# Amanda-Zheng/MR-GNAS

Measured on AMD Instinct MI355X. Metric: million edges/sec per supernet fwd+bwd step (FB15k-237, dim=200), higher is better.
Workload: dtype f32

## Files before the change

mr-gnas_amd/csrc/gemm_dispatch.hpp:

```cpp
#pragma once
#include "gemm_x3.hpp"
#include "gemm_x3s.hpp"
#include "gemm_x3s8.hpp"
#include "gemm_x3q.hpp"

namespace mrg {

inline int gemm_mode() { return gemm_switches().mode; }

constexpr int X3Q_MIN_K = 224;
inline bool x3q_shape(int epi, int N, int K) {
  const int q = gemm_switches().q;
  return gemm_mode() == 0 && q != 0 && epi != EPI_SEGMAX && epi != EPI_SEGSUM && N > 128 && N <= X3Q_NT * 16 && K > (q == 2 ? 48 : X3Q_MIN_K);
}

constexpr int X3N_NT = 2;
inline bool x3n_shape(int epi, int64_t rows, int N, int K) {
  return gemm_mode() == 0 && rows > 0 && rows <= gemm_switches().small_rows && gemm_pick_nt(N) > X3N_NT && N <= 224 && !x3q_shape(epi, N, K);
}

inline size_t bsplit_bytes_any(int N, int K) {
  const size_t a = x3_bsplit_bytes(N, K, gemm_pick_nt(N));
  const size_t q = (N > 128 && N <= X3Q_NT * 16) ? x3q_bsplit_bytes(K) : 0;
  const size_t n = (gemm_pick_nt(N) > X3N_NT && N <= 224) ? x3_bsplit_bytes(N, K, X3N_NT) : 0;
  const size_t m = a > q ? a : q;
  return m > n ? m : n;
}

inline void launch_bsplit_any(int epi, int64_t rows, const float* B, int64_t sn, int64_t sk, int N, int K, void* Bp, hipStream_t st) {
  if (x3q_shape(epi, N, K)) {
    const float* Bs[1] = {B};
    void* outs[1] = {Bp};
    launch_bsplitq3(Bs, sn, sk, N, K, outs, 1, st);
  } else {
    launch_bsplit(B, sn, sk, N, K, x3n_shape(epi, rows, N, K) ? X3N_NT : gemm_pick_nt(N), Bp, st);
  }
}
inline void launch_bsplit3_any(int epi, int64_t rows, const float* const* B, int64_t sn, int64_t sk, int N, int K, void* const* out, hipStream_t st,
                               const float* const* B2 = nullptr, int ksplit = 0) {
  if (x3q_shape(epi, N, K)) launch_bsplitq3(B, sn, sk, N, K, out, 3, st, B2, ksplit);
  else launch_bsplit3(B, sn, sk, N, K, x3n_shape(epi, rows, N, K) ? X3N_NT : gemm_pick_nt(N), out, st, B2, ksplit);
}

template <int EPI>
inline int launch_rowgemm_x3_mode(GemmArgs a, const void* Bp, hipStream_t st) {
  if (x3q_shape(EPI, a.N, a.K1 + a.K2)) {
    if (!x3q_eligible(a)) return MRG_E_SHAPE;
    return launch_rowgemm_x3q<EPI>(a, Bp, st);
  }
  if (x3n_shape(EPI, a.rows, a.N, a.K1 + a.K2)) {
    if (!x3_eligible(a)) return MRG_E_SHAPE;
    return launch_rowgemm_x3<EPI>(a, Bp, st, X3N_NT);
  }
  if (gemm_mode() != 2 && x3s_eligible(a)) {
    if constexpr (EPI != EPI_GATE) {
      if (x3s8_eligible<EPI>(a)) return launch_rowgemm_x3s8<EPI>(a, Bp, st);
    }
    return launch_rowgemm_x3s<EPI>(a, Bp, st);
  }
  return launch_rowgemm_x3<EPI>(a, Bp, st);
}

inline size_t gemm_workspace_bytes(int K, int N) {
  const size_t split = bsplit_bytes_any(N, K);
  const size_t transp = (size_t)K * N * sizeof(float);
  return split > transp ? split : transp;
}

template <int EPI>
inline int launch_gemm(GemmArgs a, int64_t b_sn, int64_t b_sk, void* ws, hipStream_t st) {
  if (a.rows <= 0) return MRG_OK;
  if (!a.A2 || a.K2 == 0) { a.A2 = a.A1; a.K2 = 0; }
  const int K = a.K1 + a.K2;
  if (ws && gemm_mode() != 1 && x3_eligible(a)) {
    launch_bsplit_any(EPI, a.rows, a.B, b_sn, b_sk, a.N, K, ws, st);
    return launch_rowgemm_x3_mode<EPI>(a, ws, st);
  }
  if (b_sk != 1) {
    if (!ws) return MRG_E_WORKSPACE;
    launch_transpose(a.B, (float*)ws, (int)(K), a.N, (int)b_sk, st);
    a.B = (const float*)ws;
    a.ldb = K;
  } else {
    a.ldb = (int)b_sn;
  }
  return launch_rowgemm<EPI>(a, st);
}

}
```

mr-gnas_amd/csrc/gemm_x3q.hpp:

```cpp
#pragma once
#include "gemm_x3.hpp"

namespace mrg {

constexpr int X3Q_CHUNK = X3Q_HT * 3 * 1024;
constexpr int X3Q_ROWS = 64;

inline size_t x3q_bsplit_bytes(int K) { return (size_t)x3q_slabs(K) * 2 * X3Q_CHUNK; }

template <int EPI>
__device__ __forceinline__ void gemm_epilogue_q(const GemmArgs& a, f32x4v (&acc)[X3Q_NT], int64_t rowbase, int li, int lh, bool full) {
  if (rowbase >= a.rows) return;
  const int last = (int)((a.rows - 1 - rowbase) < 15 ? (a.rows - 1 - rowbase) : 15);
  const int colw = li < a.N ? li : a.N - 1;
  float* crow[8];
  const float* srow[8];
  float* xrow[8];
  float cs[8];
  bool rok[8];
  const bool cstore = EPI != EPI_GATE || a.C != nullptr;
#pragma unroll
  for (int i = 0; i < 8; ++i) {
    const int row = i + 8 * lh;
    const int rc = row < last ? row : last;
    rok[i] = row <= last;
    crow[i] = a.C + (rowbase + rc) * a.ldc + colw;
    if (EPI == EPI_GATE) srow[i] = a.S + (rowbase + rc) * a.ld_s + colw;
    if (EPI == EPI_ACCUM) srow[i] = a.Cin + (rowbase + rc) * a.ld_cin + colw;
    if (EPI == EPI_GATE) xrow[i] = a.aux ? a.aux + (rowbase + rc) * a.N + colw : nullptr;
    cs[i] = 1.0f;
    if (EPI == EPI_GATE || EPI == EPI_SCALE) cs[i] = a.scale * (a.rowscale ? a.rowscale[rowbase + rc] : 1.0f);
  }
  const int lc = li & 15;
#pragma unroll
  for (int j = 0; j < X3Q_HT; ++j) {
    const int ca = (2 * j) * 16 + lc, cb = (2 * j + 1) * 16 + lc;
    const float bva = a.bias ? a.bias[ca < a.N ? ca : a.N - 1] : 0.f;
    const float bvb = a.bias ? a.bias[cb < a.N ? cb : a.N - 1] : 0.f;
    float acc8[8];
#pragma unroll
    for (int r = 0; r < 4; ++r) {
      float xa = acc[2 * j][r] + bva, xb = acc[2 * j + 1][r] + bvb;
      asm volatile("s_nop 1\n\tv_permlane16_swap_b32 %0, %1" : "+v"(xa), "+v"(xb));
      acc8[r] = xa;
      acc8[4 + r] = xb;
    }
    const int col = j * 32 + li;
    const bool cok = col < a.N;
    const int off = cok ? j * 32 : 0;
    float in[8], v[8], g[8];
#pragma unroll
    for (int i = 0; i < 8; ++i) in[i] = 0.f;
    if ((EPI == EPI_GATE && cstore) || EPI == EPI_ACCUM) {
#pragma unroll
      for (int i = 0; i < 8; ++i) in[i] = srow[i][off];
    }
#pragma unroll
    for (int i = 0; i < 8; ++i) {
      const float x = acc8[i];
      if (EPI == EPI_BIAS_ACT) {
        v[i] = (a.act == MRG_ACT_RELU) ? (x > 0.f ? x : 0.f) : (a.act == MRG_ACT_SIGMOID ? sigmoidf_fast(x) : x);
      } else if (EPI == EPI_GATE) {
        g[i] = sigmoidf_fast(x);
        v[i] = g[i] * in[i] * cs[i];
      } else if (EPI == EPI_SCALE) {
        v[i] = x * cs[i];
      } else {
        v[i] = x + in[i];
      }
    }
    if (full) {
      if (cok) {
        if (cstore) {
#pragma unroll
          for (int i = 0; i < 8; ++i) crow[i][j * 32] = v[i];
        }
        if (EPI == EPI_GATE && a.aux) {
#pragma unroll
          for (int i = 0; i < 8; ++i) xrow[i][j * 32] = g[i];
        }
      }
    } else {
#pragma unroll
      for (int i = 0; i < 8; ++i) {
        if (cok && rok[i]) {
          if (cstore) crow[i][j * 32] = v[i];
          if (EPI == EPI_GATE && a.aux) xrow[i][j * 32] = g[i];
        }
      }
    }
  }
}

constexpr int X3Q_WPS = 3;

template <int EPI, bool DUAL>
__global__ __launch_bounds__(256, X3Q_WPS) void rowgemm_x3q_k(GemmArgs a, const char* __restrict__ Bp) {
  constexpr int NCH = X3Q_HT * 3;
  constexpr int NBW = (NCH + 3) / 4;
  extern __shared__ __align__(16) char smem_q[];
  const int tid = threadIdx.x, wave = __builtin_amdgcn_readfirstlane(tid >> 6), lane = tid & 63;
  const int lr = lane & 15, lg = lane >> 4;
  MRG_GROUP_SELECT(X3Q_ROWS)
  const int64_t roww = row0 + wave * 16;
  const int K = a.K1 + a.K2;
  const int nslab = (K + 31) >> 5;

  f32x4v acc[X3Q_NT];
#pragma unroll
  for (int n = 0; n < X3Q_NT; ++n)
#pragma unroll
    for (int r = 0; r < 4; ++r) acc[n][r] = 0.f;

  const float* ar1; const float* ar2;
  x3_a_row(a, roww + lr, ar1, ar2);
  v4f xr[2][2];
  auto load_a = [&](int slab, v4f (&x)[2]) { x3_load_a<32, DUAL>(x, slab, nslab, lg, ar1, ar2, a.K1, a.K2, K); };
  auto fetch_b = [&](int c) { x3_fetch_b<NCH>(Bq + (int64_t)c * X3Q_CHUNK, smem_q + (c & 1) * X3Q_CHUNK, wave, lane); };
  const unsigned lds0 = (unsigned)(size_t)(lds_ptr_t)smem_q + (unsigned)lane * 16u;
  u32x4 bq[2][3];
  auto read_b = [&](int t, int buf, u32x4 (&q)[3]) { x3_read_b(lds0 + (unsigned)(buf * X3Q_CHUNK + t * 3072), q); };
  u32x4 ch, cm, cl, nh, nm, nl;
  load_a(0, xr[0]);
  fetch_b(0);
  fetch_b(1);
  load_a(1, xr[1]);
  asm volatile("s_waitcnt vmcnt(%0)" ::"n"(NBW + 2) : "memory");
  __builtin_amdgcn_sched_barrier(0);
#pragma unroll
  for (int q = 0; q < 4; ++q) split_pair_of(xr[0], q, ch, cm, cl);
  __builtin_amdgcn_s_barrier();

  auto half_slab = [&](auto half_c, auto split_c, const v4f (&xn)[2]) {
    constexpr int HF = decltype(half_c)::value;
    constexpr bool SPLIT = decltype(split_c)::value;
    read_b(0, HF, bq[0]);
#pragma unroll
    for (int t = 0; t < X3Q_HT; ++t) {
      if (t + 1 < X3Q_HT) {
        read_b(t + 1, HF, bq[(t + 1) & 1]);
        asm volatile("s_waitcnt lgkmcnt(3)" ::: "memory");
      } else {
        asm volatile("s_waitcnt lgkmcnt(0)" ::: "memory");
      }
      __builtin_amdgcn_sched_barrier(0);
      if (SPLIT && t < 4) split_pair_of(xn, t, nh, nm, nl);
      const bf16x8 Ah = __builtin_bit_cast(bf16x8, ch), Am = __builtin_bit_cast(bf16x8, cm), Al = __builtin_bit_cast(bf16x8, cl);
      const bf16x8 Bh = __builtin_bit_cast(bf16x8, bq[t & 1][0]), Bm = __builtin_bit_cast(bf16x8, bq[t & 1][1]), Bl = __builtin_bit_cast(bf16x8, bq[t & 1][2]);
      x3_chain(acc[HF * X3Q_HT + t], Ah, Am, Al, Bh, Bm, Bl);
      if (SPLIT) {
#pragma unroll
        for (int i = 0; i < 6; ++i) {
          __builtin_amdgcn_sched_group_barrier(0x008, 1, 0);
          __builtin_amdgcn_sched_group_barrier(0x002, 2, 0);
        }
      }
      __builtin_amdgcn_sched_barrier(0);
    }
  };

  auto slab = [&](auto r_c, int s) {
    constexpr int R = decltype(r_c)::value;
    const bool has_next = s + 1 < nslab;
    if (s > 0) fetch_b(2 * s + 1);
    half_slab(std::integral_constant<int, 0>{}, std::false_type{}, xr[0]);
    asm volatile("s_waitcnt vmcnt(0)" ::: "memory");
    __builtin_amdgcn_s_barrier();
    if (has_next) fetch_b(2 * s + 2);
    load_a(s + 2, xr[R]);
    half_slab(std::integral_constant<int, 1>{}, std::true_type{}, xr[R ^ 1]);
    ch = nh; cm = nm; cl = nl;
    if (has_next) {
      asm volatile("s_waitcnt vmcnt(2)" ::: "memory");
      __builtin_amdgcn_s_barrier();
    }
  };
  int s = 0;
  for (; s + 1 < nslab; s += 2) {
    slab(std::integral_constant<int, 0>{}, s);
    slab(std::integral_constant<int, 1>{}, s + 1);
  }
  if (s < nslab) slab(std::integral_constant<int, 0>{}, s);
  asm volatile("s_waitcnt vmcnt(0)" ::: "memory");
  asm volatile("" :: "v"(xr[0][0]), "v"(xr[0][1]), "v"(xr[1][0]), "v"(xr[1][1]));

  const int li = lane & 31, lh = lane >> 5;
  gemm_epilogue_q<EPI>(a, acc, roww, li, lh, row0 + X3Q_ROWS <= a.rows);
}

inline bool x3q_eligible(const GemmArgs& a) { return x3_eligible(a) && a.rows > 0 && a.N <= X3Q_NT * 16 && !a.row_seg; }

template <int EPI>
inline int launch_rowgemm_x3q(GemmArgs a, const void* Bp, hipStream_t st) {
  if (a.rows <= 0) return MRG_OK;
  if (!a.A2 || a.K2 == 0) { a.A2 = a.A1; a.K2 = 0; }
  const int gbm = X3Q_ROWS;
  if (a.grp.n > 0 && gemm_group_tiles(a.grp, gbm) == 0) return MRG_OK;
  dim3 grid((unsigned)(a.grp.n > 0 ? a.grp.tile0[3] : (a.rows + gbm - 1) / gbm));
  const size_t lds = (size_t)2 * X3Q_CHUNK;
  if constexpr (EPI == EPI_SEGMAX || EPI == EPI_SEGSUM) {
    return MRG_E_SHAPE;
  } else {
    if (a.K2 > 0) return launch_kernel(rowgemm_x3q_k<EPI, true>, grid, dim3(256), lds, st, a, Bp);
    return launch_kernel(rowgemm_x3q_k<EPI, false>, grid, dim3(256), lds, st, a, Bp);
  }
}

}
```

mr-gnas_amd/csrc/linear.hip:

```cpp
#include "gemm_dispatch.hpp"

namespace mrg {

constexpr int WBR = 16;

struct WgradArgs {
  const float* gY; int Nout; int ldg;
  const float* X1; const float* X2; int K1, K2;
  float* ws;
  int64_t rows, rows_per_block;
  int TM, TN, TNB;
  int ngrp;
  int64_t g_lo[3], g_hi[3], g_rpb[3], g_ws_off[3];
  int g_G[3];
};

struct XSel { const float* base; int ld, kk; };
__device__ __forceinline__ XSel wgrad_sel_x(const WgradArgs& a, int c) {
  const bool first = c < a.K1 || a.K2 == 0;
  XSel s;
  s.base = first ? a.X1 : a.X2;
  s.ld = first ? a.K1 : a.K2;
  s.kk = first ? c : c - a.K1;
  return s;
}

template <int TPW, int NPF, bool VEC4>
__global__ __launch_bounds__(MRG_BLOCK, (TPW <= 7 ? 2 : 1)) void wgrad_k(WgradArgs a) {
  extern __shared__ __align__(16) float smem[];
  const int tn0 = (int)(((int64_t)blockIdx.y * a.TN) / gridDim.y);
  const int tnb = (int)(((int64_t)(blockIdx.y + 1) * a.TN) / gridDim.y) - tn0;
  const int ldg = a.TM * 32, ldx = tnb * 32, stage = WBR * (ldg + a.TNB * 32);
  const int tid = threadIdx.x, wave = tid >> 6, lane = tid & 63, li = lane & 31, lh = lane >> 5;
  const int ntiles = a.TM * tnb;
  const int g4 = ldg / 4, x4 = ldx / 4, nf4 = WBR * (g4 + x4);
  f32x16 acc[TPW];
#pragma unroll
  for (int i = 0; i < TPW; ++i)
#pragma unroll
    for (int r = 0; r < 16; ++r) acc[i][r] = 0.f;

  const int64_t r_begin = (int64_t)blockIdx.x * a.rows_per_block;
  int64_t r_end = r_begin + a.rows_per_block;
  if (r_end > a.rows) r_end = a.rows;

  float4 pf[NPF];
  auto fetch = [&](int64_t r0) {
#pragma unroll
    for (int i = 0; i < NPF; ++i) {
      int f = tid + i * MRG_BLOCK;
      const bool isg = f < WBR * g4;
      const int f2 = isg ? f : (f < nf4 ? f - WBR * g4 : 0);
      const int per = isg ? g4 : x4;
      const int r = f2 / per, c4 = f2 - r * per;
      if (VEC4) {
        const XSel sx = wgrad_sel_x(a, tn0 * 32 + c4 * 4);
        const float* base = isg ? a.gY : sx.base;
        const int ld = isg ? a.Nout : sx.ld;
        const int kk = isg ? c4 * 4 : sx.kk;
        pf[i] = gemm_raw4<true>(base, r0 + r, r_end, kk, ld, ld);
      } else {
        const int64_t rc = r0 + r < r_end ? r0 + r : r_end - 1;
        float v[4];
#pragma unroll
        for (int j = 0; j < 4; ++j) {
          const XSel sx = wgrad_sel_x(a, tn0 * 32 + c4 * 4 + j);
          const float* base = isg ? a.gY : sx.base;
          const int ld = isg ? a.Nout : sx.ld;
          const int kk = isg ? c4 * 4 + j : sx.kk;
          v[j] = base[rc * ld + (kk < ld ? kk : ld - 1)];
        }
        pf[i] = make_float4(v[0], v[1], v[2], v[3]);
      }
    }
  };
  auto stash = [&](int buf, int64_t r0) {
    const int K = a.K1 + a.K2;
#pragma unroll
    for (int i = 0; i < NPF; ++i) {
      int f = tid + i * MRG_BLOCK;
      if (f < nf4) {
        const bool isg = f < WBR * g4;
        const int f2 = isg ? f : f - WBR * g4;
        const int per = isg ? g4 : x4;
        const int r = f2 / per, c4 = f2 - r * per;
        const int c = tn0 * 32 + c4 * 4;
        const XSel sx = wgrad_sel_x(a, c);
        float4 v;
        if (VEC4) {
          v = gemm_mask4<true>(pf[i], r0 + r, r_end, isg ? c4 * 4 : sx.kk, isg ? a.Nout : sx.ld);
        } else {
          v = gemm_mask4<false>(pf[i], r0 + r, r_end, isg ? c4 * 4 : c, isg ? a.Nout : K);
        }
        if (!isg && r0 + r < r_end) {
          if (c == K) v.x = 1.0f;
          if (!VEC4) { if (c + 1 == K) v.y = 1.0f; if (c + 2 == K) v.z = 1.0f; if (c + 3 == K) v.w = 1.0f; }
        }
        *reinterpret_cast<float4*>(&smem[buf * stage + f * 4]) = v;
      }
    }
  };

  if (r_begin < r_end) {
    fetch(r_begin);
    stash(0, r_begin);
  }
  __syncthreads();
  int cur = 0;
  for (int64_t r0 = r_begin; r0 < r_end; r0 += WBR) {
    const bool more = r0 + WBR < r_end;
    if (more) fetch(r0 + WBR);
    const float* Gs = smem + cur * stage;
    const float* Xs = Gs + WBR * ldg;
#pragma unroll 1
    for (int t = 0; t < WBR / 2; ++t) {
      const float* grow = Gs + (2 * t + lh) * ldg + li;
      const float* xrow = Xs + (2 * t + lh) * ldx + li;
#pragma unroll
      for (int i = 0; i < TPW; ++i) {
        const int id = wave + 4 * i;
        if (id < ntiles) {
          const int m = id / tnb, n = id - m * tnb;
          acc[i] = __builtin_amdgcn_mfma_f32_32x32x2f32(grow[m * 32], xrow[n * 32], acc[i], 0, 0, 0);
        }
      }
    }
    if (more) {
      stash(cur ^ 1, r0 + WBR);
      __syncthreads();
      cur ^= 1;
    }
  }
  const int ldw = a.TN * 32;
  float* out = a.ws + (int64_t)blockIdx.x * ldg * ldw;
#pragma unroll
  for (int i = 0; i < TPW; ++i) {
    const int id = wave + 4 * i;
    if (id < ntiles) {
      const int m = id / tnb, n = id - m * tnb;
#pragma unroll
      for (int r = 0; r < 16; ++r) {
        const int row = m * 32 + (r & 3) + 8 * (r >> 2) + 4 * lh;
        out[(int64_t)row * ldw + (tn0 + n) * 32 + li] = acc[i][r];
      }
    }
  }
}

static __device__ float mrg_zeros16[4] = {0.f, 0.f, 0.f, 0.f};
static __device__ float mrg_ones16[4] = {1.f, 0.f, 0.f, 0.f};

template <int TPW, int NPF>
__global__ __launch_bounds__(MRG_BLOCK, (TPW <= 7 ? 2 : 1)) void wgrad_dma_k(WgradArgs a) {
  extern __shared__ __align__(16) float smem[];
  const int tn0 = (int)(((int64_t)blockIdx.y * a.TN) / gridDim.y);
  const int tnb = (int)(((int64_t)(blockIdx.y + 1) * a.TN) / gridDim.y) - tn0;
  const int ldg = a.TM * 32, ldx = tnb * 32, stage = WBR * (ldg + a.TNB * 32);
  const int tid = threadIdx.x, wave = tid >> 6, lane = tid & 63, li = lane & 31, lh = lane >> 5;
  const int g4 = ldg / 4, x4 = ldx / 4, nf4 = WBR * (g4 + x4);
  const int K = a.K1 + a.K2;
  f32x16 acc[TPW];
#pragma unroll
  for (int i = 0; i < TPW; ++i)
#pragma unroll
    for (int r = 0; r < 16; ++r) acc[i][r] = 0.f;

  const int64_t r_begin = (int64_t)blockIdx.x * a.rows_per_block;
  int64_t r_end = r_begin + a.rows_per_block;
  if (r_end > a.rows) r_end = a.rows;

  const float* src[NPF]; int64_t stride[NPF]; int rr[NPF]; int kind[NPF];
#pragma unroll
  for (int i = 0; i < NPF; ++i) {
    const int f = tid + i * MRG_BLOCK;
    const bool isg = f < WBR * g4;
    const int f2 = isg ? f : (f < nf4 ? f - WBR * g4 : 0);
    const int per = isg ? g4 : x4;
    const int r = f2 / per, c = (f2 - r * per) * 4 + (isg ? 0 : tn0 * 32);
    rr[i] = r;
    if (isg) {
      kind[i] = c < a.Nout ? 0 : 2;
      src[i] = a.gY + (r_begin + r) * a.ldg + (c < a.Nout ? c : 0);
      stride[i] = (int64_t)WBR * a.ldg;
    } else {
      const XSel sx = wgrad_sel_x(a, c < K ? c : 0);
      kind[i] = c < K ? 0 : (c == K ? 1 : 2);
      src[i] = sx.base + (r_begin + r) * sx.ld + sx.kk;
      stride[i] = (int64_t)WBR * sx.ld;
    }
  }
  auto fetch = [&](int buf, int64_t r0, int64_t tile) {
#pragma unroll
    for (int i = 0; i < NPF; ++i) {
      const int f = tid + i * MRG_BLOCK;
      if (f - lane < nf4) {
        const bool rv = r0 + rr[i] < r_end;
        const float* p = (rv && kind[i] == 0) ? src[i] + tile * stride[i] : ((rv && kind[i] == 1) ? mrg_ones16 : mrg_zeros16);
        if (f < nf4)
          __builtin_amdgcn_global_load_lds((gbl_ptr_t)p, (lds_ptr_t)(smem + buf * stage + (f - lane) * 4), 16, 0, 0);
      }
    }
  };
  const unsigned lds0 = (unsigned)(size_t)(lds_ptr_t)smem;
  unsigned goff[TPW];
#pragma unroll
  for (int i = 0; i < TPW; ++i) goff[i] = (unsigned)((lh * ldg + (i < a.TM ? i : 0) * 32 + li) * 4);
  const unsigned xoff = (unsigned)((WBR * ldg + lh * ldx + (wave < tnb ? wave : 0) * 32 + li) * 4);
  const bool active = wave < tnb;
  int per_tile = 0;
#pragma unroll
  for (int i = 0; i < NPF; ++i) per_tile += (wave * 64 + i * MRG_BLOCK < nf4) ? 1 : 0;
  if (r_begin < r_end) fetch(0, r_begin, 0);
  if (r_begin + WBR < r_end) fetch(1, r_begin + WBR, 1);
  int cur = 0;
  int64_t tile = 0;
  for (int64_t r0 = r_begin; r0 < r_end; r0 += WBR, ++tile) {
    wait_vmcnt(r0 + WBR < r_end ? per_tile : 0);
    __builtin_amdgcn_s_barrier();
    if (r0 + 2 * WBR < r_end) fetch(cur >= 1 ? cur - 1 : 2, r0 + 2 * WBR, tile + 2);
    const unsigned base = lds0 + cur * stage * 4;
    float gv[2][TPW], xv[2];
    auto frag = [&](int b, int t) {
      asm volatile("ds_read_b32 %0, %1" : "=v"(xv[b]) : "v"(base + xoff + t * 2 * ldx * 4));
#pragma unroll
      for (int i = 0; i < TPW; ++i) asm volatile("ds_read_b32 %0, %1" : "=v"(gv[b][i]) : "v"(base + goff[i] + t * 2 * ldg * 4));
    };
    frag(0, 0);
#pragma unroll
    for (int t = 0; t < WBR / 2; ++t) {
      const int c = t & 1;
      if (t + 1 < WBR / 2) {
        frag(c ^ 1, t + 1);
        asm volatile("s_waitcnt lgkmcnt(%0)" ::"n"(TPW + 1) : "memory");
      } else {
        asm volatile("s_waitcnt lgkmcnt(0)" ::: "memory");
      }
      __builtin_amdgcn_sched_barrier(0);
      if (active) {
#pragma unroll
        for (int i = 0; i < TPW; ++i)
          if (i < a.TM) acc[i] = __builtin_amdgcn_mfma_f32_32x32x2f32(gv[c][i], xv[c], acc[i], 0, 0, 0);
      }
      __builtin_amdgcn_sched_barrier(0);
    }
    cur = cur == 2 ? 0 : cur + 1;
  }
  const int ldw = a.TN * 32;
  float* out = a.ws + (int64_t)blockIdx.x * ldg * ldw;
#pragma unroll
  for (int i = 0; i < TPW; ++i) {
    if (active && i < a.TM) {
#pragma unroll
      for (int r = 0; r < 16; ++r) {
        const int row = i * 32 + (r & 3) + 8 * (r >> 2) + 4 * lh;
        out[(int64_t)row * ldw + (tn0 + wave) * 32 + li] = acc[i][r];
      }
    }
  }
}

constexpr int WX_THREADS = 512;
constexpr int WX_APITCH = 57 * 4;

template <int NG>
__global__ __launch_bounds__(WX_THREADS, 1) void wgrad_x3_k(WgradArgs a) {
  constexpr int KP = 8 / NG, KT = 2 * KP;
  constexpr int SLOTS = NG == 2 ? 4 : 3;
  constexpr int BPITCH = (KT * 8 + 1) * 4;
  constexpr int ACH = WBR * 57, BCH = WBR * (KT * 8 + 1), STAGE_CH = ACH + BCH;
  constexpr int NPF = (STAGE_CH + WX_THREADS - 1) / WX_THREADS;
  extern __shared__ __align__(16) float smem[];
  const int tn0 = (int)(((int64_t)blockIdx.y * a.TN) / gridDim.y);
  const int tnb = (int)(((int64_t)(blockIdx.y + 1) * a.TN) / gridDim.y) - tn0;
  const int tid = threadIdx.x, wave = __builtin_amdgcn_readfirstlane(tid >> 6), lane = tid & 63, li = lane & 31, lh = lane >> 5;
  const int wg = wave / KP, wp = wave % KP;
  const int m0 = wg * 4;
  const int an = a.TM - m0 < 4 ? (a.TM - m0 > 0 ? a.TM - m0 : 0) : 4;
  const int kn = tnb - 2 * wp < 2 ? (tnb - 2 * wp > 0 ? tnb - 2 * wp : 0) : 2;
  const int K = a.K1 + a.K2;

  f32x16 acc[4][2];
#pragma unroll
  for (int i = 0; i < 4; ++i)
#pragma unroll
    for (int j = 0; j < 2; ++j)
#pragma unroll
      for (int r = 0; r < 16; ++r) acc[i][j][r] = 0.f;

  int64_t r_begin = (int64_t)blockIdx.x * a.rows_per_block;
  int64_t r_end = r_begin + a.rows_per_block;
  if (r_end > a.rows) r_end = a.rows;
  int64_t ws_off = 0;
  if (a.ngrp > 0) {
    const int z = blockIdx.z;
#define MRG_PICKZ(F) (z == 0 ? a.F[0] : (z == 1 ? a.F[1] : a.F[2]))
    if ((int)blockIdx.x >= MRG_PICKZ(g_G)) return;
    const int64_t rpb = MRG_PICKZ(g_rpb), hi = MRG_PICKZ(g_hi);
    r_begin = MRG_PICKZ(g_lo) + (int64_t)blockIdx.x * rpb;
    r_end = r_begin + rpb < hi ? r_begin + rpb : hi;
    ws_off = MRG_PICKZ(g_ws_off);
#undef MRG_PICKZ
  }

  const float* src[NPF]; int64_t stride[NPF]; int rr[NPF]; int kind[NPF];
#pragma unroll
  for (int i = 0; i < NPF; ++i) {
    const int f = tid + i * WX_THREADS;
    const bool isg = f < ACH;
    const int f2 = isg ? f : (f < STAGE_CH ? f - ACH : 0);
    const int per = isg ? 57 : KT * 8 + 1;
    const int r = f2 / per, c = (f2 - r * per) * 4;
    rr[i] = r;
    if (isg) {
      kind[i] = c < a.Nout ? 0 : 2;
      src[i] = a.gY + (r_begin + r) * a.ldg + (c < a.Nout ? c : 0);
      stride[i] = (int64_t)WBR * a.ldg;
    } else {
      const int cg = tn0 * 32 + c;
      const bool incol = c < tnb * 32;
      const XSel sx = wgrad_sel_x(a, (incol && cg < K) ? cg : 0);
      kind[i] = (incol && cg < K) ? 0 : ((incol && cg == K) ? 1 : 2);
      src[i] = sx.base + (r_begin + r) * sx.ld + sx.kk;
      stride[i] = (int64_t)WBR * sx.ld;
    }
  }
  int per_tile = 0;
#pragma unroll
  for (int i = 0; i < NPF; ++i) per_tile += (wave * 64 + i * WX_THREADS < STAGE_CH) ? 1 : 0;
  auto fetch = [&](int buf, int64_t r0, int64_t tile) {
#pragma unroll
    for (int i = 0; i < NPF; ++i) {
      const int f = tid + i * WX_THREADS;
      if (f - lane < STAGE_CH) {
        const bool rv = r0 + rr[i] < r_end;
        const float* p = (rv && kind[i] == 0) ? src[i] + tile * stride[i] : ((rv && kind[i] == 1) ? mrg_ones16 : mrg_zeros16);
        if (f < STAGE_CH)
          __builtin_amdgcn_global_load_lds((gbl_ptr_t)p, (lds_ptr_t)(smem + (buf * STAGE_CH + (f - lane)) * 4), 16, 0, 0);
      }
    }
  };

  const unsigned lds0 = (unsigned)(size_t)(lds_ptr_t)smem;
  const unsigned a_off = (unsigned)((8 * lh * WX_APITCH + m0 * 32 + li) * 4);
  const unsigned b_off = (unsigned)((ACH * 4 + 8 * lh * BPITCH + 2 * wp * 32 + li) * 4);
  auto frag = [&](unsigned addr, auto pitch_c, u32x4& H, u32x4& M, u32x4& L) {
    constexpr int PB = decltype(pitch_c)::value * 4;
    float v[8];
    asm volatile("ds_read_b32 %0, %1" : "=v"(v[0]) : "v"(addr));
    asm volatile("ds_read_b32 %0, %1 offset:%2" : "=v"(v[1]) : "v"(addr), "n"(PB));
    asm volatile("ds_read_b32 %0, %1 offset:%2" : "=v"(v[2]) : "v"(addr), "n"(2 * PB));
    asm volatile("ds_read_b32 %0, %1 offset:%2" : "=v"(v[3]) : "v"(addr), "n"(3 * PB));
    asm volatile("ds_read_b32 %0, %1 offset:%2" : "=v"(v[4]) : "v"(addr), "n"(4 * PB));
    asm volatile("ds_read_b32 %0, %1 offset:%2" : "=v"(v[5]) : "v"(addr), "n"(5 * PB));
    asm volatile("ds_read_b32 %0, %1 offset:%2" : "=v"(v[6]) : "v"(addr), "n"(6 * PB));
    asm volatile("ds_read_b32 %0, %1 offset:%2" : "=v"(v[7]) : "v"(addr), "n"(7 * PB));
    asm volatile("s_waitcnt lgkmcnt(0)" ::: "memory");
    __builtin_amdgcn_sched_barrier(0);
    split8(v, H, M, L);
  };

  if (r_begin < r_end) fetch(0, r_begin, 0);
#pragma unroll
  for (int t = 1; t < SLOTS - 1; ++t)
    if (r_begin + t * WBR < r_end) fetch(t, r_begin + t * WBR, t);
  int cur = 0;
  int64_t tile = 0;
  for (int64_t r0 = r_begin; r0 < r_end; r0 += WBR, ++tile) {
    {
      int64_t left = (r_end - r0 + WBR - 1) / WBR - 1;
      wait_vmcnt((int)(left < SLOTS - 2 ? left : SLOTS - 2) * per_tile);
    }
    __builtin_amdgcn_s_barrier();
    if (r0 + (SLOTS - 1) * WBR < r_end)
      fetch(cur == 0 ? SLOTS - 1 : cur - 1, r0 + (SLOTS - 1) * WBR, tile + SLOTS - 1);
    const unsigned base = lds0 + cur * (STAGE_CH * 16);
    if (an > 0 && kn > 0) {
      u32x4 bh[2], bm[2], bl[2];
      frag(base + b_off, std::integral_constant<int, BPITCH>{}, bh[0], bm[0], bl[0]);
      if (kn > 1) frag(base + b_off + 128, std::integral_constant<int, BPITCH>{}, bh[1], bm[1], bl[1]);
#pragma unroll
      for (int i = 0; i < 4; ++i) {
        if (i < an) {
          u32x4 ah, am, al;
          frag(base + a_off + i * 128, std::integral_constant<int, WX_APITCH>{}, ah, am, al);
          const bf16x8 Ah = __builtin_bit_cast(bf16x8, ah), Am = __builtin_bit_cast(bf16x8, am), Al = __builtin_bit_cast(bf16x8, al);
          const bf16x8 Bh0 = __builtin_bit_cast(bf16x8, bh[0]), Bm0 = __builtin_bit_cast(bf16x8, bm[0]), Bl0 = __builtin_bit_cast(bf16x8, bl[0]);
          if (kn > 1) {
            const bf16x8 Bh1 = __builtin_bit_cast(bf16x8, bh[1]), Bm1 = __builtin_bit_cast(bf16x8, bm[1]), Bl1 = __builtin_bit_cast(bf16x8, bl[1]);
            x3_chain2(acc[i][0], acc[i][1], Ah, Am, Al, Bh0, Bm0, Bl0, Ah, Am, Al, Bh1, Bm1, Bl1);
          } else {
            x3_chain(acc[i][0], Ah, Am, Al, Bh0, Bm0, Bl0);
          }
        }
      }
    }
    cur = cur == SLOTS - 1 ? 0 : cur + 1;
  }
  const int ldw = a.TN * 32;
  float* out = a.ws + ws_off + (int64_t)blockIdx.x * (a.TM * 32) * ldw;
#pragma unroll
  for (int i = 0; i < 4; ++i)
#pragma unroll
    for (int j = 0; j < 2; ++j)
      if (i < an && j < kn) {
#pragma unroll
        for (int r = 0; r < 16; ++r) {
          const int row = (m0 + i) * 32 + (r & 3) + 8 * (r >> 2) + 4 * lh;
          out[(int64_t)row * ldw + (tn0 + 2 * wp + j) * 32 + li] = acc[i][j][r];
        }
      }
}


template <int NG>
__global__ __launch_bounds__(WX_THREADS, 1) void wgrad_x3v_k(WgradArgs a) {
  constexpr int KP = 8 / NG, KT = 2 * KP;
  constexpr int ASLOTS = NG == 2 ? 8 : 4;
  constexpr int NFRAG = ASLOTS + KT;
  constexpr int FPW = (NFRAG + 7) / 8;
  extern __shared__ __align__(16) float smem[];
  const int tn0 = (int)(((int64_t)blockIdx.y * a.TN) / gridDim.y);
  const int tnb = (int)(((int64_t)(blockIdx.y + 1) * a.TN) / gridDim.y) - tn0;
  const int tid = threadIdx.x, wave = __builtin_amdgcn_readfirstlane(tid >> 6), lane = tid & 63, li = lane & 31, lh = lane >> 5;
  const int wg = wave / KP, wp = wave % KP;
  const int m0 = wg * 4;
  const int an = a.TM - m0 < 4 ? (a.TM - m0 > 0 ? a.TM - m0 : 0) : 4;
  const int kn = tnb - 2 * wp < 2 ? (tnb - 2 * wp > 0 ? tnb - 2 * wp : 0) : 2;
  const int K = a.K1 + a.K2;

  f32x16 acc[4][2];
#pragma unroll
  for (int i = 0; i < 4; ++i)
#pragma unroll
    for (int j = 0; j < 2; ++j)
#pragma unroll
      for (int r = 0; r < 16; ++r) acc[i][j][r] = 0.f;

  int64_t r_begin = (int64_t)blockIdx.x * a.rows_per_block;
  int64_t r_end = r_begin + a.rows_per_block;
  if (r_end > a.rows) r_end = a.rows;
  int64_t ws_off = 0;
  if (a.ngrp > 0) {
    const int z = blockIdx.z;
#define MRG_PICKZ(F) (z == 0 ? a.F[0] : (z == 1 ? a.F[1] : a.F[2]))
    if ((int)blockIdx.x >= MRG_PICKZ(g_G)) return;
    const int64_t rpb = MRG_PICKZ(g_rpb), hi = MRG_PICKZ(g_hi);
    r_begin = MRG_PICKZ(g_lo) + (int64_t)blockIdx.x * rpb;
    r_end = r_begin + rpb < hi ? r_begin + rpb : hi;
    ws_off = MRG_PICKZ(g_ws_off);
#undef MRG_PICKZ
  }

  const float* src[FPW]; int64_t ld[FPW]; bool live[FPW];
#pragma unroll
  for (int i = 0; i < FPW; ++i) {
    const int f = wave + 8 * i;
    live[i] = f < NFRAG && (f < ASLOTS ? f < a.TM : f - ASLOTS < tnb);
    const float* base = mrg_zeros16; int64_t l = 0;
    if (live[i]) {
      if (f < ASLOTS) {
        const int cg = f * 32 + li;
        if (cg < a.Nout) { base = a.gY + (r_begin + 8 * lh) * a.ldg + cg; l = a.ldg; }
      } else {
        const int cg = (tn0 + f - ASLOTS) * 32 + li;
        if (cg < K) {
          const XSel sx = wgrad_sel_x(a, cg);
          base = sx.base + (r_begin + 8 * lh) * sx.ld + sx.kk; l = sx.ld;
        } else if (cg == K) {
          base = mrg_ones16;
        }
      }
    }
    src[i] = base; ld[i] = l;
  }
  constexpr unsigned BUF_BYTES = FPW * 8 * 3 * 1024;

  const int64_t nfull = (r_end - r_begin) / WBR;
  const int nv_tail = (int)((r_end - r_begin) - nfull * WBR);
  const int kbase = 8 * lh;
  float raw[FPW][8];
  auto fetch = [&](int64_t t) {
    const int64_t toff = t * WBR;
#pragma unroll
    for (int i = 0; i < FPW; ++i) {
      const float* p = src[i] + toff * ld[i];
#pragma unroll
      for (int j = 0; j < 8; ++j) raw[i][j] = p[j * ld[i]];
    }
  };
  auto produce = [&](int buf, auto tail_c) {
    constexpr bool TAIL = decltype(tail_c)::value;
#pragma unroll
    for (int i = 0; i < FPW; ++i) {
      if (live[i]) {
        float x[8];
#pragma unroll
        for (int j = 0; j < 8; ++j) x[j] = (!TAIL || kbase + j < nv_tail) ? raw[i][j] : 0.f;
        u32x4 H, M, L;
        split8(x, H, M, L);
        const int f = wave + 8 * i;
        u32x4* dst = reinterpret_cast<u32x4*>(reinterpret_cast<char*>(smem) + buf * BUF_BYTES + f * 3072) + lane;
        dst[0] = H; dst[64] = M; dst[128] = L;
      }
    }
  };
  auto rdfrag = [&](int buf, int f, bf16x8& H, bf16x8& M, bf16x8& L) {
    const u32x4* p = reinterpret_cast<const u32x4*>(reinterpret_cast<const char*>(smem) + buf * BUF_BYTES + f * 3072) + lane;
    H = __builtin_bit_cast(bf16x8, p[0]); M = __builtin_bit_cast(bf16x8, p[64]); L = __builtin_bit_cast(bf16x8, p[128]);
  };
  auto consume = [&](int cur) {
    if (an > 0 && kn > 0) {
      bf16x8 Bh0, Bm0, Bl0, Bh1, Bm1, Bl1;
      rdfrag(cur, ASLOTS + 2 * wp, Bh0, Bm0, Bl0);
      if (kn > 1) rdfrag(cur, ASLOTS + 2 * wp + 1, Bh1, Bm1, Bl1);
      else { Bh1 = Bh0; Bm1 = Bm0; Bl1 = Bl0; }
      bf16x8 An[3];
      rdfrag(cur, m0, An[0], An[1], An[2]);
#pragma unroll
      for (int i = 0; i < 4; ++i) {
        if (i < an) {
          const bf16x8 Ah = An[0], Am = An[1], Al = An[2];
          if (i + 1 < an) rdfrag(cur, m0 + i + 1, An[0], An[1], An[2]);
          if (kn > 1) {
            x3_chain2(acc[i][0], acc[i][1], Ah, Am, Al, Bh0, Bm0, Bl0, Ah, Am, Al, Bh1, Bm1, Bl1);
          } else {
            x3_chain(acc[i][0], Ah, Am, Al, Bh0, Bm0, Bl0);
          }
        }
      }
    }
  };

  if (nfull > 0) {
    fetch(0);
    produce(0, std::false_type{});
    fetch(nfull > 1 ? 1 : 0);
    __syncthreads();
    int cur = 0;
    for (int64_t t = 0; t < nfull; ++t) {
      consume(cur);
      if (t + 1 < nfull) produce(cur ^ 1, std::false_type{});
      fetch(t + 2 < nfull ? t + 2 : nfull - 1);
      __syncthreads();
      cur ^= 1;
    }
  }
  if (nv_tail > 0) {
    const int64_t toff = nfull * WBR;
#pragma unroll
    for (int i = 0; i < FPW; ++i) {
      const float* p = src[i] + toff * ld[i];
#pragma unroll
      for (int j = 0; j < 8; ++j) raw[i][j] = p[(int64_t)(kbase + j >= nv_tail ? j - WBR : j) * ld[i]];
    }
    produce(0, std::true_type{});
    __syncthreads();
    consume(0);
  }
  const int ldw = a.TN * 32;
  float* out = a.ws + ws_off + (int64_t)blockIdx.x * (a.TM * 32) * ldw;
#pragma unroll
  for (int i = 0; i < 4; ++i)
#pragma unroll
    for (int j = 0; j < 2; ++j)
      if (i < an && j < kn) {
#pragma unroll
        for (int r = 0; r < 16; ++r) {
          const int row = (m0 + i) * 32 + (r & 3) + 8 * (r >> 2) + 4 * lh;
          out[(int64_t)row * ldw + (tn0 + 2 * wp + j) * 32 + li] = acc[i][j][r];
        }
      }
}

template <int NG>
static int launch_wgrad_x3(dim3 grid, const WgradArgs& a, hipStream_t st) {
  const int kt = 16 / NG;
  bool v1 = gemm_switches().wgrad_variant == 1 && a.rows >= WBR;
  for (int i = 0; i < a.ngrp; ++i) v1 = v1 && !(a.g_hi[i] > a.g_lo[i] && a.g_hi[i] < WBR);
  if (v1) return launch_kernel(wgrad_x3v_k<NG>, grid, dim3(WX_THREADS), (size_t)2 * ((((NG == 2 ? 8 : 4) + kt) + 7) / 8 * 8) * 3 * 1024, st, a);
  return launch_kernel(wgrad_x3_k<NG>, grid, dim3(WX_THREADS), (size_t)(NG == 2 ? 4 : 3) * WBR * (57 + kt * 8 + 1) * 16, st, a);
}

struct WgradReduce3 { const float* ws[3]; float* gW[3]; float* gbias[3]; int G[3]; };
__global__ void wgrad_reduce3_k(WgradReduce3 p, int K, int Nout, int ldg, int ldx) {
  __shared__ float part[16][64];
  const int z = blockIdx.z;
  const float* __restrict__ ws = z == 0 ? p.ws[0] : (z == 1 ? p.ws[1] : p.ws[2]);
  float* __restrict__ gW = z == 0 ? p.gW[0] : (z == 1 ? p.gW[1] : p.gW[2]);
  float* __restrict__ gbias = z == 0 ? p.gbias[0] : (z == 1 ? p.gbias[1] : p.gbias[2]);
  const int G = z == 0 ? p.G[0] : (z == 1 ? p.G[1] : p.G[2]);
  if (!gW) return;
  const int tx = threadIdx.x & 63, ty = threadIdx.x >> 6;
  const int c = blockIdx.x * 64 + tx;
  const int n = blockIdx.y;
  float acc = 0.f;
  if (c <= K)
    for (int g = ty; g < G; g += 16) acc += ws[((int64_t)g * ldg + n) * ldx + c];
  part[ty][tx] = acc;
  __syncthreads();
  if (ty == 0 && c <= K) {
    float tot = part[0][tx];
#pragma unroll
    for (int i = 1; i < 16; ++i) tot += part[i][tx];
    if (c < K) gW[(int64_t)n * K + c] = tot;
    else if (gbias) gbias[n] = tot;
  }
}

struct WgradPlan {
  int TM, TN, TNB, tpw, npf, G;
  int64_t rows_per_block;
  size_t lds;
  bool ok;
};

constexpr int WGRAD_SHARE_MAX_BLOCKS = 400;

static WgradPlan wgrad_plan(int64_t rows, int K, int Nout, bool dma = false, int share = 1) {
  WgradPlan p{};
  p.TM = (Nout + 31) / 32;
  p.TN = (K + 1 + 31) / 32;
  const int opts[] = {1, 2, 4, 7, 13};
  p.tpw = 0;
  if (dma && p.TM <= 7) {
    p.TNB = p.TN < 4 ? p.TN : 4;
    for (int o : opts) if (p.TM <= o) { p.tpw = o; break; }
  } else {
    p.TNB = p.TM * p.TN <= 28 ? p.TN : (28 / p.TM > 0 ? 28 / p.TM : 0);
    int per_wave = p.TNB > 0 ? (p.TM * p.TNB + 3) / 4 : 99;
    for (int o : opts) if (per_wave <= o) { p.tpw = o; break; }
  }
  int nf4 = WBR * (p.TM + p.TNB) * 8;
  p.npf = (nf4 + MRG_BLOCK - 1) / MRG_BLOCK;
  p.lds = (size_t)(dma ? 3 : 2) * WBR * (p.TM + p.TNB) * 32 * sizeof(float);
  p.ok = p.tpw > 0 && p.lds <= 160 * 1024 && p.npf <= 16;
  int64_t tiles = (rows + WBR - 1) / WBR;
  const int ny = (p.TN + (p.TM <= 4 ? 16 : 8) - 1) / (p.TM <= 4 ? 16 : 8);
  const bool shared = share > 1 && (tiles + 15) / 16 <= WGRAD_SHARE_MAX_BLOCKS;
  const int64_t gshare = 256 / (ny * share);
  const int64_t gmax = !shared ? (256 / ny > 32 ? 256 / ny : 32) : (gshare > 16 ? gshare : 16);
  int64_t G = (tiles + 15) / 16 < gmax ? (tiles + 15) / 16 : gmax;
  const int64_t gsmall = (tiles + 3) / 4 < 8 ? (tiles + 3) / 4 : 8;
  if (G < gsmall) G = gsmall;
  if (G < 1) G = 1;
  int64_t tpb = (tiles + G - 1) / G;
  if (tpb < 1) tpb = 1;
  p.rows_per_block = tpb * WBR;
  p.G = (int)((rows + p.rows_per_block - 1) / p.rows_per_block);
  if (p.G < 1) p.G = 1;
  return p;
}

int64_t wgrad_workspace_bytes(int64_t rows, int K, int Nout) {
  WgradPlan p = wgrad_plan(rows, K, Nout);
  return (int64_t)p.G * p.TM * 32 * p.TN * 32 * sizeof(float);
}

static int launch_wgrad_one(const float* gY, int ldg, const float* X1, const float* X2, int K1, int K2, float* gW, float* gbias, void* ws,
                           int64_t rows, int Nout, int share, hipStream_t st);

static int launch_wgrad(const float* gY, const float* X1, const float* X2, int K1, int K2, float* gW, float* gbias, void* ws,
                        int64_t rows, int Nout, int share, hipStream_t st) {
  const bool splittable = Nout > 224 && rows > 0 && (Nout % 4 == 0) && (K1 % 4 == 0) && (K2 % 4 == 0) && aligned16(gY) && aligned16(X1) &&
                          (!X2 || K2 == 0 || aligned16(X2)) && K1 >= 4 && (K2 == 0 || K2 >= 4);
  if (splittable) {
    const int nblk = (Nout + 223) / 224;
    const int cw = (((Nout + nblk - 1) / nblk) + 31) / 32 * 32;
    for (int n0 = 0; n0 < Nout; n0 += cw) {
      const int nc = Nout - n0 < cw ? Nout - n0 : cw;
      int rc = launch_wgrad_one(gY + n0, Nout, X1, X2, K1, K2, gW + (int64_t)n0 * (K1 + K2), gbias ? gbias + n0 : nullptr, ws, rows, nc, share, st);
      if (rc != MRG_OK) return rc;
    }
    return MRG_OK;
  }
  return launch_wgrad_one(gY, Nout, X1, X2, K1, K2, gW, gbias, ws, rows, Nout, share, st);
}

static int launch_wgrad_one(const float* gY, int ldg, const float* X1, const float* X2, int K1, int K2, float* gW, float* gbias, void* ws,
                           int64_t rows, int Nout, int share, hipStream_t st) {
  const int K = K1 + K2;
  if (rows == 0) {
    hipError_t e = hipMemsetAsync(gW, 0, sizeof(float) * (size_t)Nout * K, st);
    if (e == hipSuccess && gbias) e = hipMemsetAsync(gbias, 0, sizeof(float) * (size_t)Nout, st);
    return (int)e;
  }
  const bool vec0 = (Nout % 4 == 0) && (K1 % 4 == 0) && (K2 % 4 == 0) && aligned16(gY) && aligned16(X1) && (!X2 || K2 == 0 || aligned16(X2)) &&
                    Nout >= 4 && K1 >= 4 && (K2 == 0 || K2 >= 4) && Nout <= 224;
  WgradPlan p = wgrad_plan(rows, K, Nout, vec0, share);
  if (!p.ok) return MRG_E_SHAPE;
  WgradArgs a{};
  a.gY = gY; a.Nout = Nout; a.ldg = ldg; a.X1 = X1; a.X2 = X2; a.K1 = K1; a.K2 = K2; a.ws = (float*)ws;
  a.rows = rows; a.rows_per_block = p.rows_per_block; a.TM = p.TM; a.TN = p.TN; a.TNB = p.TNB;
  if (!X2 || K2 == 0) { a.X2 = X1; a.K2 = 0; }
  const bool vec = vec0;
  if (vec && gemm_mode() != 1 && p.TM <= 7) {
    const int ng = p.TM <= 4 ? 1 : 2, kt = 16 / ng;
    dim3 gridx(p.G, (p.TN + kt - 1) / kt);
    const int rcx = ng == 1 ? launch_wgrad_x3<1>(gridx, a, st) : launch_wgrad_x3<2>(gridx, a, st);
    if (rcx != MRG_OK) return rcx;
    WgradReduce3 red{};
    red.ws[0] = (const float*)ws; red.gW[0] = gW; red.gbias[0] = gbias; red.G[0] = p.G;
    hipLaunchKernelGGL(wgrad_reduce3_k, dim3((K + 1 + 63) / 64, Nout, 1), dim3(1024), 0, st, red, K, Nout, p.TM * 32, p.TN * 32);
    MRG_LAUNCH_CHECK();
    return MRG_OK;
  }
  dim3 grid(p.G, (p.TN + p.TNB - 1) / p.TNB);
#define GO(T, F)                                                                                                       \
  do {                                                                                                                 \
    if (vec) {                                                                                                         \
      (void)hipFuncSetAttribute(reinterpret_cast<const void*>(&wgrad_dma_k<T, F>), hipFuncAttributeMaxDynamicSharedMemorySize, (int)p.lds); \
      hipLaunchKernelGGL((wgrad_dma_k<T, F>), grid, dim3(MRG_BLOCK), p.lds, st, a);                                    \
    } else {                                                                                                           \
      (void)hipFuncSetAttribute(reinterpret_cast<const void*>(&wgrad_k<T, F, false>), hipFuncAttributeMaxDynamicSharedMemorySize, (int)p.lds); \
      hipLaunchKernelGGL((wgrad_k<T, F, false>), grid, dim3(MRG_BLOCK), p.lds, st, a);                                 \
    }                                                                                                                  \
  } while (0)
#define GOF(T)                                                                                                         \
  do {                                                                                                                 \
    if (p.npf <= 2) GO(T, 2); else if (p.npf <= 4) GO(T, 4); else if (p.npf <= 8) GO(T, 8); else GO(T, 16);            \
  } while (0)
  switch (p.tpw) {
    case 1: GOF(1); break;
    case 2: GOF(2); break;
    case 4: GOF(4); break;
    case 7: GOF(7); break;
    default: GOF(13); break;
  }
#undef GOF
#undef GO
  MRG_LAUNCH_CHECK();
  WgradReduce3 red1{};
  red1.ws[0] = (const float*)ws; red1.gW[0] = gW; red1.gbias[0] = gbias; red1.G[0] = p.G;
  hipLaunchKernelGGL(wgrad_reduce3_k, dim3((K + 1 + 63) / 64, Nout, 1), dim3(1024), 0, st, red1, K, Nout, p.TM * 32, p.TN * 32);
  MRG_LAUNCH_CHECK();
  return MRG_OK;
}

__global__ void segmax_finalize_k(const unsigned long long* __restrict__ keys, const float* __restrict__ self_rows,
                                  const int32_t* __restrict__ eid, float* __restrict__ out, int32_t* __restrict__ arg,
                                  float* __restrict__ mx, int64_t total) {
  for (int64_t i = (int64_t)blockIdx.x * blockDim.x + threadIdx.x; i < total; i += (int64_t)gridDim.x * blockDim.x) {
    const unsigned long long k = keys[i];
    const unsigned lo = (unsigned)k;
    const float v = __uint_as_float((unsigned)(k >> 32));
    out[i] = self_rows ? v + self_rows[i] : v;
    if (arg) arg[i] = lo == 0u ? -1 : eid[0xFFFFFFFFu - lo];
    if (mx) mx[i] = v;
  }
}

}

using namespace mrg;

static bool segmax_shape_ok(int K, int Nout) { return K > 48 && K % 4 == 0 && Nout > 0; }

extern "C" int64_t mrg_linear_relu_segmax_workspace_bytes(int64_t N, int K, int Nout) {
  if (N < 0 || !segmax_shape_ok(K, Nout) || gemm_mode() == 1) return 0;
  return ((N * (int64_t)Nout * 8 + 255) / 256) * 256 + (int64_t)bsplit_bytes_any(Nout, K) + 256;
}

extern "C" int mrg_linear_relu_segmax_fwd(const float* X, const float* W, const float* bias, const int32_t* eid, const int32_t* dst,
                                          const float* self_rows, float* out, int32_t* arg, float* mx, void* ws, int64_t E, int64_t N,
                                          int K, int Nout, void* stream) {
  if (E < 0 || N < 0 || K <= 0 || Nout <= 0 || E >= ((int64_t)1 << 32) - 1) return MRG_E_SHAPE;
  if (!segmax_shape_ok(K, Nout)) return MRG_E_SHAPE;
  if (N == 0) return MRG_OK;
  if (!out || !W) return MRG_E_NULLPTR;
  if (E > 0 && (!X || !eid || !dst)) return MRG_E_NULLPTR;
  if (!ws) return MRG_E_WORKSPACE;
  if (!aligned16(X) || !aligned16(ws)) return MRG_E_SHAPE;
  hipStream_t st = (hipStream_t)stream;
  unsigned long long* keys = (unsigned long long*)ws;
  const size_t key_bytes = (size_t)((N * (int64_t)Nout * 8 + 255) / 256) * 256;
  void* bsplit = (char*)ws + key_bytes;
  if (hipMemsetAsync(keys, 0, (size_t)N * Nout * 8, st) != hipSuccess) return MRG_E_WORKSPACE;
  if (E > 0) {
    GemmArgs a{};
    a.A1 = X; a.K1 = K; a.B = W; a.bias = bias; a.N = Nout; a.rows = E; a.act = MRG_ACT_RELU;
    a.row_index = eid; a.row_seg = dst; a.seg_out = keys;
    if (!x3_eligible(a)) return MRG_E_SHAPE;
    launch_bsplit_any(EPI_SEGMAX, E, W, K, 1, Nout, K, bsplit, st);
    const int rc = launch_rowgemm_x3_mode<EPI_SEGMAX>(a, bsplit, st);
    if (rc != MRG_OK) return rc;
  }
  const int64_t total = N * (int64_t)Nout;
  hipLaunchKernelGGL(segmax_finalize_k, dim3(stream_grid_for(total, 256 * 4)), dim3(256), 0, st, keys, self_rows, eid, out, arg, mx, total);
  MRG_LAUNCH_CHECK();
  return MRG_OK;
}

extern "C" int mrg_linear_relu_segsum_fwd(const float* X, const float* W, const float* bias, const int32_t* eid, const int32_t* dst,
                                          float* part, unsigned* relu_bits, void* ws, int64_t E, int K, int Nout, void* stream) {
  if (E < 0 || K <= 0 || Nout <= 0 || E >= ((int64_t)1 << 31)) return MRG_E_SHAPE;
  if (!segmax_shape_ok(K, Nout)) return MRG_E_SHAPE;
  if (E == 0) return MRG_OK;
  if (!X || !W || !eid || !dst || !part) return MRG_E_NULLPTR;
  if (!ws) return MRG_E_WORKSPACE;
  if (!aligned16(X) || !aligned16(ws)) return MRG_E_SHAPE;
  hipStream_t st = (hipStream_t)stream;
  GemmArgs a{};
  a.A1 = X; a.K1 = K; a.B = W; a.bias = bias; a.N = Nout; a.rows = E; a.act = MRG_ACT_RELU;
  a.row_index = eid; a.row_seg = dst; a.seg_part = part; a.relu_bits = relu_bits; a.bits_ld = (Nout + 31) / 32;
  if (!x3_eligible(a)) return MRG_E_SHAPE;
  launch_bsplit_any(EPI_SEGSUM, E, W, K, 1, Nout, K, ws, st);
  return launch_rowgemm_x3_mode<EPI_SEGSUM>(a, ws, st);
}

extern "C" int64_t mrg_gemm_workspace_bytes(int K, int Nout) {
  if (K <= 0 || Nout <= 0) return 0;
  return (int64_t)gemm_workspace_bytes(K, Nout);
}

extern "C" int mrg_gemm_set_mode(int mode) {
  if (mode < 0 || mode > 2) return MRG_E_ENUM;
  gemm_switches().mode = mode;
  return MRG_OK;
}

extern "C" int mrg_wgrad_set_variant(int variant) {
  if (variant != 0 && variant != 1) return MRG_E_ENUM;
  gemm_switches().wgrad_variant = variant;
  return MRG_OK;
}

extern "C" int mrg_gemm_set_wide8(int on) {
  if (on < 0 || on > 2) return MRG_E_ENUM;
  gemm_switches().wide8 = on;
  return MRG_OK;
}

extern "C" int mrg_gemm_set_small(int on) {
  if (on < 0) return MRG_E_ENUM;
  gemm_switches().small_rows = on == 1 ? X3N_MAX_ROWS : (int64_t)on;
  return MRG_OK;
}

extern "C" int mrg_gemm_set_q(int on) {
  if (on < 0 || on > 2) return MRG_E_ENUM;
  gemm_switches().q = on;
  return MRG_OK;
}

extern "C" int mrg_gemm_set_epilogue(int mode) {
  if (mode < 0 || mode > 2) return MRG_E_ENUM;
  gemm_switches().epilogue = mode;
  return MRG_OK;
}

extern "C" int mrg_linear_fwd(const float* X, const float* W, const float* bias, float* Y, void* ws, int64_t rows, int K, int Nout,
                              int act, void* stream) {
  if (rows < 0 || K <= 0 || Nout <= 0) return MRG_E_SHAPE;
  if (act != MRG_ACT_NONE && act != MRG_ACT_RELU && act != MRG_ACT_SIGMOID) return MRG_E_ENUM;
  if (rows == 0) return MRG_OK;
  if (!X || !W || !Y) return MRG_E_NULLPTR;
  GemmArgs a{};
  a.A1 = X; a.K1 = K; a.B = W; a.bias = bias; a.C = Y; a.ldc = Nout; a.N = Nout; a.rows = rows; a.act = act;
  return launch_gemm<EPI_BIAS_ACT>(a, K, 1, ws, (hipStream_t)stream);
}

extern "C" int64_t mrg_linear_bwd_input_workspace_bytes(int K, int Nout) {
  if (K <= 0 || Nout <= 0) return 0;
  return (int64_t)gemm_workspace_bytes(Nout, K);
}

extern "C" int mrg_linear_bwd_input(const float* gY, const float* W, float* gX, void* ws, int64_t rows, int K, int Nout,
                                    int ldw, int accumulate, void* stream) {
  if (rows < 0 || K <= 0 || Nout <= 0 || ldw < K) return MRG_E_SHAPE;
  if (rows == 0) return MRG_OK;
  if (!gY || !W || !gX) return MRG_E_NULLPTR;
  if (!ws) return MRG_E_WORKSPACE;
  hipStream_t st = (hipStream_t)stream;
  GemmArgs a{};
  a.A1 = gY; a.K1 = Nout; a.B = W; a.C = gX; a.ldc = K; a.N = K; a.rows = rows; a.act = MRG_ACT_NONE;
  if (accumulate) {
    a.Cin = gX; a.ld_cin = K;
    return launch_gemm<EPI_ACCUM>(a, 1, ldw, ws, st);
  }
  return launch_gemm<EPI_BIAS_ACT>(a, 1, ldw, ws, st);
}

static size_t bwd_input3_each(int K, int Nout) { return (size_t)(((int64_t)bsplit_bytes_any(K, Nout) + 255) / 256 * 256); }

extern "C" int64_t mrg_linear_bwd_input3_workspace_bytes(int K, int Nout) {
  if (K <= 0 || Nout <= 48 || Nout % 4 != 0 || gemm_mode() == 1) return 0;
  return 3 * (int64_t)bwd_input3_each(K, Nout);
}

extern "C" int mrg_linear_bwd_input3(const float* gY, const float* const* W_host, float* gX, void* ws, int64_t b0, int64_t b1, int64_t M,
                                     int K, int Nout, int ldw, int accumulate, void* stream) {
  if (K <= 0 || Nout <= 0 || ldw < K || M < 0 || b0 < 0 || b1 < b0 || M < b1) return MRG_E_SHAPE;
  if (K <= 0 || Nout <= 48 || Nout % 4 != 0) return MRG_E_SHAPE;
  if (M == 0) return MRG_OK;
  if (!gY || !W_host || !gX) return MRG_E_NULLPTR;
  if (!ws) return MRG_E_WORKSPACE;
  hipStream_t st = (hipStream_t)stream;
  GemmArgs a{};
  a.A1 = gY; a.K1 = Nout; a.C = gX; a.ldc = K; a.N = K; a.rows = M; a.act = MRG_ACT_NONE;
  if (accumulate) { a.Cin = gX; a.ld_cin = K; }
  if (!x3_eligible(a)) return MRG_E_SHAPE;
  const int64_t lo[3] = {0, b0, b1}, hi[3] = {b0, b1, M};
  const size_t each = bwd_input3_each(K, Nout);
  const float* Bs[3]; void* outs[3];
  a.grp.n = 3;
  a.grp.bp_stride = (int64_t)each;
  for (int i = 0; i < 3; ++i) {
    const bool live = hi[i] > lo[i];
    if (live && !W_host[i]) return MRG_E_NULLPTR;
    Bs[i] = live ? W_host[i] : nullptr;
    outs[i] = (char*)ws + i * each;
    a.grp.lo[i] = lo[i]; a.grp.hi[i] = live ? hi[i] : lo[i];
    a.grp.scale[i] = 1.0f;
  }
  launch_bsplit3_any(accumulate ? EPI_ACCUM : EPI_BIAS_ACT, M, Bs, 1, ldw, K, Nout, outs, st);
  MRG_LAUNCH_CHECK();
  if (accumulate) return launch_rowgemm_x3_mode<EPI_ACCUM>(a, outs[0], st);
  return launch_rowgemm_x3_mode<EPI_BIAS_ACT>(a, outs[0], st);
}

static size_t bwd_input3_pair_each(int K, int Nout) { return (size_t)(((int64_t)bsplit_bytes_any(K, 2 * Nout) + 255) / 256 * 256); }

extern "C" int64_t mrg_linear_bwd_input3_pair_workspace_bytes(int K, int Nout) {
  if (K <= 0 || Nout <= 24 || Nout % 4 != 0 || gemm_mode() == 1) return 0;
  return 3 * (int64_t)bwd_input3_pair_each(K, Nout);
}

extern "C" int mrg_linear_bwd_input3_pair(const float* gY1, const float* gY2, const float* const* W1_host, const float* const* W2_host, float* gX,
                                          void* ws, int64_t b0, int64_t b1, int64_t M, int K, int Nout, int ldw, int accumulate, void* stream) {
  if (K <= 0 || Nout <= 24 || Nout % 4 != 0 || ldw < K || M < 0 || b0 < 0 || b1 < b0 || M < b1) return MRG_E_SHAPE;
  if (M == 0) return MRG_OK;
  if (!gY1 || !gY2 || !W1_host || !W2_host || !gX) return MRG_E_NULLPTR;
  if (!ws) return MRG_E_WORKSPACE;
  hipStream_t st = (hipStream_t)stream;
  GemmArgs a{};
  a.A1 = gY1; a.K1 = Nout; a.A2 = gY2; a.K2 = Nout; a.C = gX; a.ldc = K; a.N = K; a.rows = M; a.act = MRG_ACT_NONE;
  if (accumulate) { a.Cin = gX; a.ld_cin = K; }
  if (!x3_eligible(a)) return MRG_E_SHAPE;
  const int64_t lo[3] = {0, b0, b1}, hi[3] = {b0, b1, M};
  const size_t each = bwd_input3_pair_each(K, Nout);
  const float* Bs[3]; const float* Bs2[3]; void* outs[3];
  a.grp.n = 3;
  a.grp.bp_stride = (int64_t)each;
  for (int i = 0; i < 3; ++i) {
    const bool live = hi[i] > lo[i];
    if (live && (!W1_host[i] || !W2_host[i])) return MRG_E_NULLPTR;
    Bs[i] = live ? W1_host[i] : nullptr;
    Bs2[i] = live ? W2_host[i] : nullptr;
    outs[i] = (char*)ws + i * each;
    a.grp.lo[i] = lo[i]; a.grp.hi[i] = live ? hi[i] : lo[i];
    a.grp.scale[i] = 1.0f;
  }
  launch_bsplit3_any(accumulate ? EPI_ACCUM : EPI_BIAS_ACT, M, Bs, 1, ldw, K, 2 * Nout, outs, st, Bs2, Nout);
  MRG_LAUNCH_CHECK();
  if (accumulate) return launch_rowgemm_x3_mode<EPI_ACCUM>(a, outs[0], st);
  return launch_rowgemm_x3_mode<EPI_BIAS_ACT>(a, outs[0], st);
}

static bool wgrad3_ok(int K1, int K2, int Nout) {
  return Nout >= 4 && Nout <= 224 && Nout % 4 == 0 && K1 >= 4 && K1 % 4 == 0 && K2 >= 0 && K2 % 4 == 0;
}

extern "C" int64_t mrg_linear_bwd_weight3_workspace_bytes(int64_t b0, int64_t b1, int64_t M, int K1, int K2, int Nout) {
  if (M < 0 || b0 < 0 || b1 < b0 || M < b1 || !wgrad3_ok(K1, K2, Nout) || gemm_mode() == 1) return 0;
  const int64_t rows[3] = {b0, b1 - b0, M - b1};
  int64_t total = 0;
  for (int i = 0; i < 3; ++i) total += (wgrad_workspace_bytes(rows[i], K1 + K2, Nout) + 255) / 256 * 256;
  return total;
}

extern "C" int mrg_linear_bwd_weight3(const float* gY, const float* X1, const float* X2, float* const* gW_host, float* const* gb_host, void* ws,
                                      int64_t b0, int64_t b1, int64_t M, int K1, int K2, int Nout, void* stream) {
  if (M < 0 || b0 < 0 || b1 < b0 || M < b1 || !wgrad3_ok(K1, K2, Nout)) return MRG_E_SHAPE;
  if (!gW_host) return MRG_E_NULLPTR;
  if (M > 0 && (!gY || !X1 || (K2 > 0 && !X2))) return MRG_E_NULLPTR;
  if (!ws) return MRG_E_WORKSPACE;
  if (!aligned16(gY) || !aligned16(X1) || (K2 > 0 && !aligned16(X2))) return MRG_E_SHAPE;
  hipStream_t st = (hipStream_t)stream;
  const int K = K1 + K2;
  const int64_t lo[3] = {0, b0, b1}, hi[3] = {b0, b1, M};
  WgradArgs a{};
  a.gY = gY; a.Nout = Nout; a.ldg = Nout; a.X1 = X1; a.X2 = K2 > 0 ? X2 : X1; a.K1 = K1; a.K2 = K2; a.ws = (float*)ws; a.rows = M;
  a.ngrp = 3;
  WgradReduce3 red{};
  int maxG = 0;
  int64_t off = 0;
  WgradPlan p0 = wgrad_plan(1, K, Nout, true);
  if (!p0.ok || p0.TM > 7) return MRG_E_SHAPE;
  a.TM = p0.TM; a.TN = p0.TN; a.TNB = p0.TNB;
  int nlive = 0;
  for (int i = 0; i < 3; ++i) nlive += (gW_host[i] != nullptr && hi[i] > lo[i]) ? 1 : 0;
  if (nlive < 1) nlive = 1;
  for (int i = 0; i < 3; ++i) {
    const int64_t rows = hi[i] - lo[i];
    WgradPlan p = wgrad_plan(rows, K, Nout, true, nlive);
    const bool live = gW_host[i] != nullptr;
    a.g_lo[i] = lo[i]; a.g_hi[i] = hi[i]; a.g_rpb[i] = p.rows_per_block; a.g_G[i] = live ? p.G : 0; a.g_ws_off[i] = off / (int64_t)sizeof(float);
    red.ws[i] = (const float*)((const char*)ws + off); red.gW[i] = gW_host[i]; red.gbias[i] = gb_host ? gb_host[i] : nullptr; red.G[i] = p.G;
    off += (wgrad_workspace_bytes(rows, K, Nout) + 255) / 256 * 256;
    if (live && p.G > maxG) maxG = p.G;
  }
  if (maxG == 0) return MRG_OK;
  const int ng = a.TM <= 4 ? 1 : 2, kt = 16 / ng;
  dim3 gridx(maxG, (a.TN + kt - 1) / kt, 3);
  const int rcx = ng == 1 ? launch_wgrad_x3<1>(gridx, a, st) : launch_wgrad_x3<2>(gridx, a, st);
  if (rcx != MRG_OK) return rcx;
  hipLaunchKernelGGL(wgrad_reduce3_k, dim3((K + 1 + 63) / 64, Nout, 3), dim3(1024), 0, st, red, K, Nout, a.TM * 32, a.TN * 32);
  MRG_LAUNCH_CHECK();
  return MRG_OK;
}

extern "C" int64_t mrg_linear_bwd_weight_workspace_bytes(int64_t rows, int K, int Nout) {
  if (rows < 0 || K <= 0 || Nout <= 0) return 0;
  return wgrad_workspace_bytes(rows, K, Nout);
}

extern "C" int mrg_linear_bwd_weight_share(const float* gY, const float* X1, const float* X2, float* gW, float* gbias, void* ws,
                                           int64_t rows, int K1, int K2, int Nout, int share, void* stream) {
  if (rows < 0 || K1 <= 0 || K2 < 0 || Nout <= 0) return MRG_E_SHAPE;
  if (share < 1 || share > 3) return MRG_E_ENUM;
  if (!gW) return MRG_E_NULLPTR;
  if (rows > 0 && (!gY || !X1 || (K2 > 0 && !X2))) return MRG_E_NULLPTR;
  if (rows > 0 && !ws) return MRG_E_WORKSPACE;
  return launch_wgrad(gY, X1, K2 > 0 ? X2 : nullptr, K1, K2, gW, gbias, ws, rows, Nout, share, (hipStream_t)stream);
}

extern "C" int mrg_linear_bwd_weight(const float* gY, const float* X1, const float* X2, float* gW, float* gbias, void* ws,
                                     int64_t rows, int K1, int K2, int Nout, void* stream) {
  return mrg_linear_bwd_weight_share(gY, X1, X2, gW, gbias, ws, rows, K1, K2, Nout, 1, stream);
}
```

mr-gnas_amd/csrc/x3_parts.hpp:

```cpp
#pragma once
#include <type_traits>
#include "gemm.hpp"

namespace mrg {

typedef __bf16 bf16x8 __attribute__((ext_vector_type(8)));
typedef __bf16 bf16x2 __attribute__((ext_vector_type(2)));
typedef float f32x2 __attribute__((ext_vector_type(2)));
typedef float f32x4v __attribute__((ext_vector_type(4)));
typedef unsigned u32x4 __attribute__((ext_vector_type(4)));

constexpr int64_t X3N_MAX_ROWS = 16384;
struct GemmSwitches {
  int mode = 0;
  int q = 1;
  int64_t small_rows = X3N_MAX_ROWS;
  int wide8 = 1;
  int epilogue = 0;
  int wgrad_variant = 1;
};
inline GemmSwitches& gemm_switches() { static GemmSwitches s; return s; }

__device__ __forceinline__ float sub1(float a, float b) {
  float r;
  asm("v_sub_f32 %0, %1, %2" : "=v"(r) : "v"(a), "v"(b));
  return r;
}
__device__ __forceinline__ void split_pair(float x0, float x1, unsigned& h, unsigned& m, unsigned& l) {
  f32x2 v = {x0, x1};
  h = __builtin_bit_cast(unsigned, __builtin_convertvector(v, bf16x2));
  f32x2 r = {sub1(x0, __builtin_bit_cast(float, h << 16)), sub1(x1, __builtin_bit_cast(float, h & 0xffff0000u))};
  m = __builtin_bit_cast(unsigned, __builtin_convertvector(r, bf16x2));
  f32x2 r2 = {sub1(r.x, __builtin_bit_cast(float, m << 16)), sub1(r.y, __builtin_bit_cast(float, m & 0xffff0000u))};
  l = __builtin_bit_cast(unsigned, __builtin_convertvector(r2, bf16x2));
}
__device__ __forceinline__ void split8(const float (&v)[8], u32x4& H, u32x4& M, u32x4& L) {
#pragma unroll
  for (int j = 0; j < 4; ++j) {
    unsigned h, m, l;
    split_pair(v[2 * j], v[2 * j + 1], h, m, l);
    H[j] = h; M[j] = m; L[j] = l;
  }
}
__device__ __forceinline__ void split_pair_of(const v4f (&x)[2], int q, u32x4& H, u32x4& M, u32x4& L) {
  const v4f& v = x[q >> 1];
  unsigned h, m, l;
  if (q & 1) split_pair(v.z, v.w, h, m, l); else split_pair(v.x, v.y, h, m, l);
  H[q] = h; M[q] = m; L[q] = l;
}

template <bool TR>
__device__ __forceinline__ f32x16 x3_mm(bf16x8 a, bf16x8 b, f32x16 c) {
  if constexpr (TR) return __builtin_amdgcn_mfma_f32_32x32x16_bf16(b, a, c, 0, 0, 0);
  else return __builtin_amdgcn_mfma_f32_32x32x16_bf16(a, b, c, 0, 0, 0);
}
template <bool TR>
__device__ __forceinline__ f32x4v x3_mm(bf16x8 a, bf16x8 b, f32x4v c) {
  static_assert(!TR, "the 16 x 16 x 32 kernel has no transposed form");
  return __builtin_amdgcn_mfma_f32_16x16x32_bf16(a, b, c, 0, 0, 0);
}
template <bool TR = false, class ACC>
__device__ __forceinline__ void x3_chain(ACC& c, bf16x8 Ah, bf16x8 Am, bf16x8 Al, bf16x8 Bh, bf16x8 Bm, bf16x8 Bl) {
  c = x3_mm<TR>(Am, Bm, c);
  c = x3_mm<TR>(Al, Bh, c);
  c = x3_mm<TR>(Ah, Bl, c);
  c = x3_mm<TR>(Am, Bh, c);
  c = x3_mm<TR>(Ah, Bm, c);
  c = x3_mm<TR>(Ah, Bh, c);
}
template <bool TR = false>
__device__ __forceinline__ void x3_chain2(f32x16& c0, f32x16& c1, bf16x8 Ah0, bf16x8 Am0, bf16x8 Al0, bf16x8 Bh0, bf16x8 Bm0, bf16x8 Bl0,
                                          bf16x8 Ah1, bf16x8 Am1, bf16x8 Al1, bf16x8 Bh1, bf16x8 Bm1, bf16x8 Bl1) {
  c0 = x3_mm<TR>(Am0, Bm0, c0); c1 = x3_mm<TR>(Am1, Bm1, c1);
  c0 = x3_mm<TR>(Al0, Bh0, c0); c1 = x3_mm<TR>(Al1, Bh1, c1);
  c0 = x3_mm<TR>(Ah0, Bl0, c0); c1 = x3_mm<TR>(Ah1, Bl1, c1);
  c0 = x3_mm<TR>(Am0, Bh0, c0); c1 = x3_mm<TR>(Am1, Bh1, c1);
  c0 = x3_mm<TR>(Ah0, Bm0, c0); c1 = x3_mm<TR>(Ah1, Bm1, c1);
  c0 = x3_mm<TR>(Ah0, Bh0, c0); c1 = x3_mm<TR>(Ah1, Bh1, c1);
}
template <bool TR = false, int MT, int NT>
__device__ __forceinline__ void x3_chain_rows(f32x16 (&acc)[MT][NT], int n, const u32x4 (&Ah)[MT], const u32x4 (&Am)[MT], const u32x4 (&Al)[MT],
                                              bf16x8 Bh, bf16x8 Bm, bf16x8 Bl) {
  static_assert(MT == 1 || MT == 2, "one or two row tiles per wave");
  auto c = [](const u32x4& v) { return __builtin_bit_cast(bf16x8, v); };
  if constexpr (MT == 2) x3_chain2<TR>(acc[0][n], acc[1][n], c(Ah[0]), c(Am[0]), c(Al[0]), Bh, Bm, Bl, c(Ah[1]), c(Am[1]), c(Al[1]), Bh, Bm, Bl);
  else x3_chain<TR>(acc[0][n], c(Ah[0]), c(Am[0]), c(Al[0]), Bh, Bm, Bl);
}

inline int x3_tiles(int N, int nt) { return ((N + nt * 32 - 1) / (nt * 32)) * nt; }
inline int x3_slabs(int K) { return (K + 15) / 16; }
inline size_t x3_bsplit_bytes(int N, int K, int nt) { return (size_t)x3_slabs(K) * x3_tiles(N, nt) * 3 * 64 * 16; }
struct BSplitTiles32 {
  static __host__ __device__ int chunks(int ntile, int nslab) { return nslab * ntile * 64; }
  static __host__ __device__ int tiles(int ntile, int) { return ntile; }
  static __device__ __forceinline__ void source(int lane, int tile, int slab, int& n, int& k0) {
    n = tile * 32 + (lane & 31); k0 = slab * 16 + (lane >> 5) * 8;
  }
};
constexpr int X3Q_HT = 7;
constexpr int X3Q_NT = 2 * X3Q_HT;
struct BSplitTiles16 {
  static __host__ __device__ int chunks(int nslab) { return nslab * X3Q_NT * 64; }
  static __host__ __device__ int tiles(int) { return X3Q_NT; }
  static __device__ __forceinline__ void source(int lane, int tile, int slab, int& n, int& k0) {
    n = tile * 16 + (lane & 15); k0 = slab * 32 + (lane >> 4) * 8;
  }
};
struct BSplit3 { const float* B[3]; u32x4* out[3]; const float* B2[3]; int ksplit; };
template <class LAYOUT, class... DIMS>
static __global__ void bsplit_k(BSplit3 p, int64_t sn, int64_t sk, int N, int K, DIMS... dims) {
  const float* __restrict__ B = p.B[blockIdx.y];
  const float* __restrict__ B2 = p.B2[blockIdx.y];
  const int ksplit = (p.ksplit > 0 && B2) ? p.ksplit : K;
  u32x4* __restrict__ Bp = p.out[blockIdx.y];
  if (!B) return;
  const int idx = blockIdx.x * blockDim.x + threadIdx.x;
  if (idx >= LAYOUT::chunks(dims...)) return;
  const int ntile = LAYOUT::tiles(dims...);
  const int lane = idx & 63, tile = (idx >> 6) % ntile, slab = (idx >> 6) / ntile;
  int n, k0;
  LAYOUT::source(lane, tile, slab, n, k0);
  float v[8];
#pragma unroll
  for (int j = 0; j < 8; ++j) {
    const int k = k0 + j;
    v[j] = (n < N && k < K) ? (k < ksplit ? B[n * sn + k * sk] : B2[n * sn + (k - ksplit) * sk]) : 0.f;
  }
  u32x4 h, m, l;
#pragma unroll
  for (int j = 0; j < 4; ++j) {
    unsigned a, b, c;
    split_pair(v[2 * j], v[2 * j + 1], a, b, c);
    h[j] = a; m[j] = b; l[j] = c;
  }
  u32x4* o = Bp + ((int64_t)(slab * ntile + tile) * 3) * 64 + lane;
  o[0] = h; o[64] = m; o[128] = l;
}
template <class LAYOUT, class... DIMS>
inline void launch_bsplit_layout(const float* const* B, int64_t sn, int64_t sk, int N, int K, void* const* out, int count, hipStream_t st,
                                 const float* const* B2, int ksplit, DIMS... dims) {
  BSplit3 p{};
  for (int i = 0; i < count; ++i) { p.B[i] = B[i]; p.out[i] = (u32x4*)out[i]; p.B2[i] = B2 ? B2[i] : nullptr; }
  p.ksplit = B2 ? ksplit : 0;
  hipLaunchKernelGGL((bsplit_k<LAYOUT, DIMS...>), dim3((LAYOUT::chunks(dims...) + 255) / 256, count), dim3(256), 0, st, p, sn, sk, N, K, dims...);
}
inline void launch_bsplit3(const float* const* B, int64_t sn, int64_t sk, int N, int K, int nt, void* const* out, hipStream_t st,
                           const float* const* B2 = nullptr, int ksplit = 0) {
  const int ntile = x3_tiles(N, nt), nslab = x3_slabs(K);
  launch_bsplit_layout<BSplitTiles32>(B, sn, sk, N, K, out, 3, st, B2, ksplit, ntile, nslab);
}
inline void launch_bsplit(const float* B, int64_t sn, int64_t sk, int N, int K, int nt, void* Bp, hipStream_t st) {
  const int ntile = x3_tiles(N, nt), nslab = x3_slabs(K);
  launch_bsplit_layout<BSplitTiles32>(&B, sn, sk, N, K, &Bp, 1, st, nullptr, 0, ntile, nslab);
}
inline int x3q_slabs(int K) { return (K + 31) / 32; }
inline void launch_bsplitq3(const float* const* B, int64_t sn, int64_t sk, int N, int K, void* const* out, int count, hipStream_t st,
                            const float* const* B2 = nullptr, int ksplit = 0) {
  const int nslab = x3q_slabs(K);
  launch_bsplit_layout<BSplitTiles16>(B, sn, sk, N, K, out, count, st, B2, ksplit, nslab);
}

__device__ __forceinline__ void wait_vmcnt(int n) {
#define MRG_VM(N) case N: asm volatile("s_waitcnt vmcnt(" #N ")" ::: "memory"); break;
  switch (n) {
    MRG_VM(0) MRG_VM(1) MRG_VM(2) MRG_VM(3) MRG_VM(4) MRG_VM(5) MRG_VM(6) MRG_VM(7)
    MRG_VM(8) MRG_VM(9) MRG_VM(10) MRG_VM(11) MRG_VM(12) MRG_VM(13) MRG_VM(14) MRG_VM(15)
    MRG_VM(16) MRG_VM(17) MRG_VM(18) MRG_VM(19) MRG_VM(20) MRG_VM(21) MRG_VM(22) MRG_VM(23)
    MRG_VM(24) MRG_VM(25) MRG_VM(26) MRG_VM(27) MRG_VM(28) MRG_VM(29) MRG_VM(30) MRG_VM(31)
    MRG_VM(32) MRG_VM(33) MRG_VM(34) MRG_VM(35) MRG_VM(36) MRG_VM(37) MRG_VM(38) MRG_VM(39)
    MRG_VM(40) MRG_VM(41) MRG_VM(42) MRG_VM(43) MRG_VM(44) MRG_VM(45) MRG_VM(46) MRG_VM(47)
    MRG_VM(48) MRG_VM(49) MRG_VM(50) MRG_VM(51) MRG_VM(52) MRG_VM(53) MRG_VM(54) MRG_VM(55)
    MRG_VM(56) MRG_VM(57) MRG_VM(58) MRG_VM(59) MRG_VM(60) MRG_VM(61) MRG_VM(62)
    default: asm volatile("s_waitcnt vmcnt(63)" ::: "memory"); break;
  }
#undef MRG_VM
}

#define MRG_PICK(F) (sg == 0 ? a.grp.F[0] : (sg == 1 ? a.grp.F[1] : a.grp.F[2]))
#define MRG_GROUP_SELECT(GBM)                                                                                          \
  int64_t row0 = (int64_t)blockIdx.x * (GBM);                                                                          \
  int sg = 0;                                                                                                          \
  if (a.grp.n > 0) sg = ((int)blockIdx.x >= a.grp.tile0[1] ? 1 : 0) + ((int)blockIdx.x >= a.grp.tile0[2] ? 1 : 0);     \
  sg = __builtin_amdgcn_readfirstlane(sg);                                                                             \
  const char* __restrict__ Bq = Bp + (int64_t)sg * a.grp.bp_stride;                                                    \
  if (a.grp.n > 0) {                \
    row0 = MRG_PICK(lo) + (int64_t)((int)blockIdx.x - MRG_PICK(tile0)) * (GBM);                                        \
    a.rows = MRG_PICK(hi);                                                                                             \
    a.bias = MRG_PICK(bias);                                                                                           \
    a.scale = MRG_PICK(scale);                                                                                         \
    if (!MRG_PICK(use_rowscale)) a.rowscale = nullptr;                                                                 \
  }

__device__ __forceinline__ void x3_a_row(const GemmArgs& a, int64_t row, const float*& ar1, const float*& ar2) {
  int64_t rc = row < a.rows ? row : a.rows - 1;
  if (rc < 0) rc = 0;
  if (a.row_index) rc = a.row_index[rc];
  ar1 = a.A1 + rc * a.K1;
  ar2 = a.A2 + rc * a.K2;
}
template <int KSLAB, bool DUAL>
__device__ __forceinline__ void x3_load_a(v4f (&x)[2], int slab, int nslab, int kg, const float* ar1, const float* ar2, int K1, int K2, int K) {
  const int sl = slab < nslab ? slab : nslab - 1;
  const int k = sl * KSLAB + kg * 8;
  const float* p0 = gemm_a_ptr<DUAL>(ar1, ar2, K1, K2, K, k);
  const float* p1 = gemm_a_ptr<DUAL>(ar1, ar2, K1, K2, K, k + 4);
  asm volatile("global_load_dwordx4 %0, %1, off" : "=v"(x[0]) : "v"(p0));
  asm volatile("global_load_dwordx4 %0, %1, off" : "=v"(x[1]) : "v"(p1));
}
template <int NCH>
__device__ __forceinline__ void x3_fetch_b(const char* __restrict__ src, char* __restrict__ dst, const int& wave, const int& lane) {
  constexpr int NBW = (NCH + 3) / 4;
#pragma unroll
  for (int i = 0; i < NBW; ++i) {
    int c = wave * NBW + i;
    c = c < NCH ? c : NCH - 1;
    __builtin_amdgcn_global_load_lds((gbl_ptr_t)(src + c * 1024 + lane * 16), (lds_ptr_t)(dst + c * 1024), 16, 0, 0);
  }
}
__device__ __forceinline__ void x3_read_b(unsigned ad, u32x4 (&q)[3]) {
  asm volatile("ds_read_b128 %0, %1" : "=v"(q[0]) : "v"(ad));
  asm volatile("ds_read_b128 %0, %1 offset:1024" : "=v"(q[1]) : "v"(ad));
  asm volatile("ds_read_b128 %0, %1 offset:2048" : "=v"(q[2]) : "v"(ad));
}

template <class... KARGS, class... ARGS>
inline int launch_kernel(void (*kernel)(KARGS...), dim3 grid, dim3 block, size_t lds, hipStream_t st, ARGS... args) {
  (void)hipFuncSetAttribute(reinterpret_cast<const void*>(kernel), hipFuncAttributeMaxDynamicSharedMemorySize, (int)lds);
  hipLaunchKernelGGL(kernel, grid, block, lds, st, static_cast<KARGS>(args)...);
  hipError_t e = hipGetLastError();
  return e == hipSuccess ? MRG_OK : (int)e;
}

}
```

Measured before the change: 11.30.

## Trim x3q GEMM to 13 tiles for N=200 and table-driven wgrad wave mapping

The x3q row GEMM is templated on tile count, so N=200 uses 13 sixteen-column tiles instead of padding to 14. This cuts B-split bytes, LDS use and MFMA work for the padded tile, and the epilogue handles an odd final tile. Separately, the weight-gradient kernels replace the fixed wave-to-(m,n) tile assignment with a precomputed per-shape lookup table. The table spreads partial tiles across waves to balance load when tile counts do not divide evenly. Risks are added complexity, a table-indexing dependency on TM and tnb bounds, and wave-divergent fragment reloads.

Result: no change. 11.33, median of 4 (+0.3%).

```diff
diff --git a/mr-gnas_amd/csrc/gemm_dispatch.hpp b/mr-gnas_amd/csrc/gemm_dispatch.hpp
--- a/mr-gnas_amd/csrc/gemm_dispatch.hpp
+++ b/mr-gnas_amd/csrc/gemm_dispatch.hpp
@@ -21,7 +21,7 @@
 
 inline size_t bsplit_bytes_any(int N, int K) {
   const size_t a = x3_bsplit_bytes(N, K, gemm_pick_nt(N));
-  const size_t q = (N > 128 && N <= X3Q_NT * 16) ? x3q_bsplit_bytes(K) : 0;
+  const size_t q = (N > 128 && N <= X3Q_NT * 16) ? x3q_bsplit_bytes(N, K) : 0;
   const size_t n = (gemm_pick_nt(N) > X3N_NT && N <= 224) ? x3_bsplit_bytes(N, K, X3N_NT) : 0;
   const size_t m = a > q ? a : q;
   return m > n ? m : n;
diff --git a/mr-gnas_amd/csrc/gemm_x3q.hpp b/mr-gnas_amd/csrc/gemm_x3q.hpp
--- a/mr-gnas_amd/csrc/gemm_x3q.hpp
+++ b/mr-gnas_amd/csrc/gemm_x3q.hpp
@@ -4,12 +4,13 @@
 namespace mrg {
 
 constexpr int X3Q_CHUNK = X3Q_HT * 3 * 1024;
-constexpr int X3Q_ROWS = 64;
-
-inline size_t x3q_bsplit_bytes(int K) { return (size_t)x3q_slabs(K) * 2 * X3Q_CHUNK; }
-
-template <int EPI>
-__device__ __forceinline__ void gemm_epilogue_q(const GemmArgs& a, f32x4v (&acc)[X3Q_NT], int64_t rowbase, int li, int lh, bool full) {
+constexpr int X3Q_WAVES = 4;
+constexpr int X3Q_ROWS = 16 * X3Q_WAVES;
+
+inline size_t x3q_bsplit_bytes(int N, int K) { return (size_t)x3q_slabs(K) * x3q_tiles(N) * 3 * 1024; }
+
+template <int EPI, int NT>
+__device__ __forceinline__ void gemm_epilogue_q(const GemmArgs& a, f32x4v (&acc)[NT], int64_t rowbase, int li, int lh, bool full) {
   if (rowbase >= a.rows) return;
   const int last = (int)((a.rows - 1 - rowbase) < 15 ? (a.rows - 1 - rowbase) : 15);
   const int colw = li < a.N ? li : a.N - 1;
@@ -33,14 +34,15 @@
   }
   const int lc = li & 15;
 #pragma unroll
-  for (int j = 0; j < X3Q_HT; ++j) {
+  for (int j = 0; j < (NT + 1) / 2; ++j) {
     const int ca = (2 * j) * 16 + lc, cb = (2 * j + 1) * 16 + lc;
     const float bva = a.bias ? a.bias[ca < a.N ? ca : a.N - 1] : 0.f;
-    const float bvb = a.bias ? a.bias[cb < a.N ? cb : a.N - 1] : 0.f;
+    const bool hasb = 2 * j + 1 < NT;
+    const float bvb = (hasb && a.bias) ? a.bias[cb < a.N ? cb : a.N - 1] : 0.f;
     float acc8[8];
 #pragma unroll
     for (int r = 0; r < 4; ++r) {
-      float xa = acc[2 * j][r] + bva, xb = acc[2 * j + 1][r] + bvb;
+      float xa = acc[2 * j][r] + bva, xb = hasb ? acc[hasb ? 2 * j + 1 : 0][r] + bvb : 0.f;
       asm volatile("s_nop 1\n\tv_permlane16_swap_b32 %0, %1" : "+v"(xa), "+v"(xb));
       acc8[r] = xa;
       acc8[4 + r] = xb;
@@ -94,10 +96,13 @@
 
 constexpr int X3Q_WPS = 3;
 
-template <int EPI, bool DUAL>
-__global__ __launch_bounds__(256, X3Q_WPS) void rowgemm_x3q_k(GemmArgs a, const char* __restrict__ Bp) {
-  constexpr int NCH = X3Q_HT * 3;
-  constexpr int NBW = (NCH + 3) / 4;
+template <int EPI, bool DUAL, int NT>
+__global__ __launch_bounds__(64 * X3Q_WAVES, X3Q_WPS) void rowgemm_x3q_k(GemmArgs a, const char* __restrict__ Bp) {
+  constexpr int HT1 = NT - X3Q_HT;
+  static_assert(HT1 >= 4 && HT1 <= X3Q_HT, "the second half-slab: at most seven tiles, at least the four the next slab's split hides behind");
+  constexpr int NCH0 = X3Q_HT * 3, NCH1 = HT1 * 3;
+  constexpr int NBW1 = (NCH1 + X3Q_WAVES - 1) / X3Q_WAVES;
+  constexpr int SLAB = NT * 3 * 1024;
   extern __shared__ __align__(16) char smem_q[];
   const int tid = threadIdx.x, wave = __builtin_amdgcn_readfirstlane(tid >> 6), lane = tid & 63;
   const int lr = lane & 15, lg = lane >> 4;
@@ -106,9 +111,9 @@
   const int K = a.K1 + a.K2;
   const int nslab = (K + 31) >> 5;
 
-  f32x4v acc[X3Q_NT];
-#pragma unroll
-  for (int n = 0; n < X3Q_NT; ++n)
+  f32x4v acc[NT];
+#pragma unroll
+  for (int n = 0; n < NT; ++n)
 #pragma unroll
     for (int r = 0; r < 4; ++r) acc[n][r] = 0.f;
 
@@ -116,16 +121,21 @@
   x3_a_row(a, roww + lr, ar1, ar2);
   v4f xr[2][2];
   auto load_a = [&](int slab, v4f (&x)[2]) { x3_load_a<32, DUAL>(x, slab, nslab, lg, ar1, ar2, a.K1, a.K2, K); };
-  auto fetch_b = [&](int c) { x3_fetch_b<NCH>(Bq + (int64_t)c * X3Q_CHUNK, smem_q + (c & 1) * X3Q_CHUNK, wave, lane); };
+  auto fetch_b = [&](auto half_c, int s) {
+    if constexpr (decltype(half_c)::value == 0) x3_fetch_b<NCH0, X3Q_WAVES>(Bq + (int64_t)s * SLAB, smem_q, wave, lane);
+    else x3_fetch_b<NCH1, X3Q_WAVES>(Bq + (int64_t)s * SLAB + X3Q_CHUNK, smem_q + X3Q_CHUNK, wave, lane);
+  };
+  constexpr std::integral_constant<int, 0> H0{};
+  constexpr std::integral_constant<int, 1> H1{};
   const unsigned lds0 = (unsigned)(size_t)(lds_ptr_t)smem_q + (unsigned)lane * 16u;
   u32x4 bq[2][3];
   auto read_b = [&](int t, int buf, u32x4 (&q)[3]) { x3_read_b(lds0 + (unsigned)(buf * X3Q_CHUNK + t * 3072), q); };
   u32x4 ch, cm, cl, nh, nm, nl;
   load_a(0, xr[0]);
-  fetch_b(0);
-  fetch_b(1);
+  fetch_b(H0, 0);
+  fetch_b(H1, 0);
   load_a(1, xr[1]);
-  asm volatile("s_waitcnt vmcnt(%0)" ::"n"(NBW + 2) : "memory");
+  asm volatile("s_waitcnt vmcnt(%0)" ::"n"(NBW1 + 2) : "memory");
   __builtin_amdgcn_sched_barrier(0);
 #pragma unroll
   for (int q = 0; q < 4; ++q) split_pair_of(xr[0], q, ch, cm, cl);
@@ -134,10 +144,11 @@
   auto half_slab = [&](auto half_c, auto split_c, const v4f (&xn)[2]) {
     constexpr int HF = decltype(half_c)::value;
     constexpr bool SPLIT = decltype(split_c)::value;
+    constexpr int HTN = HF == 0 ? X3Q_HT : HT1;
     read_b(0, HF, bq[0]);
 #pragma unroll
-    for (int t = 0; t < X3Q_HT; ++t) {
-      if (t + 1 < X3Q_HT) {
+    for (int t = 0; t < HTN; ++t) {
+      if (t + 1 < HTN) {
         read_b(t + 1, HF, bq[(t + 1) & 1]);
         asm volatile("s_waitcnt lgkmcnt(3)" ::: "memory");
       } else {
@@ -162,11 +173,11 @@
   auto slab = [&](auto r_c, int s) {
     constexpr int R = decltype(r_c)::value;
     const bool has_next = s + 1 < nslab;
-    if (s > 0) fetch_b(2 * s + 1);
+    if (s > 0) fetch_b(H1, s);
     half_slab(std::integral_constant<int, 0>{}, std::false_type{}, xr[0]);
     asm volatile("s_waitcnt vmcnt(0)" ::: "memory");
     __builtin_amdgcn_s_barrier();
-    if (has_next) fetch_b(2 * s + 2);
+    if (has_next) fetch_b(H0, s + 1);
     load_a(s + 2, xr[R]);
     half_slab(std::integral_constant<int, 1>{}, std::true_type{}, xr[R ^ 1]);
     ch = nh; cm = nm; cl = nl;
@@ -185,7 +196,7 @@
   asm volatile("" :: "v"(xr[0][0]), "v"(xr[0][1]), "v"(xr[1][0]), "v"(xr[1][1]));
 
   const int li = lane & 31, lh = lane >> 5;
-  gemm_epilogue_q<EPI>(a, acc, roww, li, lh, row0 + X3Q_ROWS <= a.rows);
+  gemm_epilogue_q<EPI, NT>(a, acc, roww, li, lh, row0 + X3Q_ROWS <= a.rows);
 }
 
 inline bool x3q_eligible(const GemmArgs& a) { return x3_eligible(a) && a.rows > 0 && a.N <= X3Q_NT * 16 && !a.row_seg; }
@@ -197,13 +208,19 @@
   const int gbm = X3Q_ROWS;
   if (a.grp.n > 0 && gemm_group_tiles(a.grp, gbm) == 0) return MRG_OK;
   dim3 grid((unsigned)(a.grp.n > 0 ? a.grp.tile0[3] : (a.rows + gbm - 1) / gbm));
-  const size_t lds = (size_t)2 * X3Q_CHUNK;
+  const int nt = x3q_tiles(a.N);
+  const size_t lds = (size_t)nt * 3 * 1024;
   if constexpr (EPI == EPI_SEGMAX || EPI == EPI_SEGSUM) {
     return MRG_E_SHAPE;
   } else {
-    if (a.K2 > 0) return launch_kernel(rowgemm_x3q_k<EPI, true>, grid, dim3(256), lds, st, a, Bp);
-    return launch_kernel(rowgemm_x3q_k<EPI, false>, grid, dim3(256), lds, st, a, Bp);
-  }
-}
-
-}
+    static_assert(X3Q_NT_MIN == 13 && X3Q_NT == 14, "one instance per tile count x3q_tiles can return");
+    if (nt == 13) {
+      if (a.K2 > 0) return launch_kernel(rowgemm_x3q_k<EPI, true, 13>, grid, dim3(64 * X3Q_WAVES), lds, st, a, Bp);
+      return launch_kernel(rowgemm_x3q_k<EPI, false, 13>, grid, dim3(64 * X3Q_WAVES), lds, st, a, Bp);
+    }
+    if (a.K2 > 0) return launch_kernel(rowgemm_x3q_k<EPI, true, 14>, grid, dim3(64 * X3Q_WAVES), lds, st, a, Bp);
+    return launch_kernel(rowgemm_x3q_k<EPI, false, 14>, grid, dim3(64 * X3Q_WAVES), lds, st, a, Bp);
+  }
+}
+
+}
diff --git a/mr-gnas_amd/csrc/linear.hip b/mr-gnas_amd/csrc/linear.hip
--- a/mr-gnas_amd/csrc/linear.hip
+++ b/mr-gnas_amd/csrc/linear.hip
@@ -1,6 +1,8 @@
 #include "gemm_dispatch.hpp"
 
 namespace mrg {
+#define WGRAD_MAP_STORAGE static __device__ const
+#include "wgrad_map.hpp"
 
 constexpr int WBR = 16;
 
@@ -273,10 +275,10 @@
   const int tn0 = (int)(((int64_t)blockIdx.y * a.TN) / gridDim.y);
   const int tnb = (int)(((int64_t)(blockIdx.y + 1) * a.TN) / gridDim.y) - tn0;
   const int tid = threadIdx.x, wave = __builtin_amdgcn_readfirstlane(tid >> 6), lane = tid & 63, li = lane & 31, lh = lane >> 5;
-  const int wg = wave / KP, wp = wave % KP;
-  const int m0 = wg * 4;
-  const int an = a.TM - m0 < 4 ? (a.TM - m0 > 0 ? a.TM - m0 : 0) : 4;
-  const int kn = tnb - 2 * wp < 2 ? (tnb - 2 * wp > 0 ? tnb - 2 * wp : 0) : 2;
+  const unsigned wm = tnb > 0 ? wgrad_map[a.TM - 1][tnb - 1][wave] : 0u;
+  const int m0 = (int)(wm & 7u), an = (int)(wm >> 3 & 7u), c0 = (int)(wm >> 6 & 15u);
+  auto wm_has = [&](int i) { return (wm >> (10 + i) & 1u) != 0; };
+  auto wm_c1 = [&](int i) { return (int)(wm >> (14 + 4 * i) & 15u); };
   const int K = a.K1 + a.K2;
 
   f32x16 acc[4][2];
@@ -342,7 +344,7 @@
 
   const unsigned lds0 = (unsigned)(size_t)(lds_ptr_t)smem;
   const unsigned a_off = (unsigned)((8 * lh * WX_APITCH + m0 * 32 + li) * 4);
-  const unsigned b_off = (unsigned)((ACH * 4 + 8 * lh * BPITCH + 2 * wp * 32 + li) * 4);
+  const unsigned b_off = (unsigned)((ACH * 4 + 8 * lh * BPITCH + li) * 4);
   auto frag = [&](unsigned addr, auto pitch_c, u32x4& H, u32x4& M, u32x4& L) {
     constexpr int PB = decltype(pitch_c)::value * 4;
     float v[8];
@@ -374,18 +376,23 @@
     if (r0 + (SLOTS - 1) * WBR < r_end)
       fetch(cur == 0 ? SLOTS - 1 : cur - 1, r0 + (SLOTS - 1) * WBR, tile + SLOTS - 1);
     const unsigned base = lds0 + cur * (STAGE_CH * 16);
-    if (an > 0 && kn > 0) {
+    if (an > 0) {
       u32x4 bh[2], bm[2], bl[2];
-      frag(base + b_off, std::integral_constant<int, BPITCH>{}, bh[0], bm[0], bl[0]);
-      if (kn > 1) frag(base + b_off + 128, std::integral_constant<int, BPITCH>{}, bh[1], bm[1], bl[1]);
+      frag(base + b_off + c0 * 128, std::integral_constant<int, BPITCH>{}, bh[0], bm[0], bl[0]);
+      bh[1] = bh[0]; bm[1] = bm[0]; bl[1] = bl[0];
+      int c1 = -1;
 #pragma unroll
       for (int i = 0; i < 4; ++i) {
         if (i < an) {
           u32x4 ah, am, al;
           frag(base + a_off + i * 128, std::integral_constant<int, WX_APITCH>{}, ah, am, al);
+          if (wm_has(i) && wm_c1(i) != c1) {
+            c1 = wm_c1(i);
+            frag(base + b_off + c1 * 128, std::integral_constant<int, BPITCH>{}, bh[1], bm[1], bl[1]);
+          }
           const bf16x8 Ah = __builtin_bit_cast(bf16x8, ah), Am = __builtin_bit_cast(bf16x8, am), Al = __builtin_bit_cast(bf16x8, al);
           const bf16x8 Bh0 = __builtin_bit_cast(bf16x8, bh[0]), Bm0 = __builtin_bit_cast(bf16x8, bm[0]), Bl0 = __builtin_bit_cast(bf16x8, bl[0]);
-          if (kn > 1) {
+          if (wm_has(i)) {
             const bf16x8 Bh1 = __builtin_bit_cast(bf16x8, bh[1]), Bm1 = __builtin_bit_cast(bf16x8, bm[1]), Bl1 = __builtin_bit_cast(bf16x8, bl[1]);
             x3_chain2(acc[i][0], acc[i][1], Ah, Am, Al, Bh0, Bm0, Bl0, Ah, Am, Al, Bh1, Bm1, Bl1);
           } else {
@@ -402,11 +409,12 @@
   for (int i = 0; i < 4; ++i)
 #pragma unroll
     for (int j = 0; j < 2; ++j)
-      if (i < an && j < kn) {
+      if (i < an && (j == 0 || wm_has(i))) {
+        const int ct = tn0 + (j == 0 ? c0 : wm_c1(i));
 #pragma unroll
         for (int r = 0; r < 16; ++r) {
           const int row = (m0 + i) * 32 + (r & 3) + 8 * (r >> 2) + 4 * lh;
-          out[(int64_t)row * ldw + (tn0 + 2 * wp + j) * 32 + li] = acc[i][j][r];
+          out[(int64_t)row * ldw + ct * 32 + li] = acc[i][j][r];
         }
       }
 }
@@ -422,10 +430,10 @@
   const int tn0 = (int)(((int64_t)blockIdx.y * a.TN) / gridDim.y);
   const int tnb = (int)(((int64_t)(blockIdx.y + 1) * a.TN) / gridDim.y) - tn0;
   const int tid = threadIdx.x, wave = __builtin_amdgcn_readfirstlane(tid >> 6), lane = tid & 63, li = lane & 31, lh = lane >> 5;
-  const int wg = wave / KP, wp = wave % KP;
-  const int m0 = wg * 4;
-  const int an = a.TM - m0 < 4 ? (a.TM - m0 > 0 ? a.TM - m0 : 0) : 4;
-  const int kn = tnb - 2 * wp < 2 ? (tnb - 2 * wp > 0 ? tnb - 2 * wp : 0) : 2;
+  const unsigned wm = tnb > 0 ? wgrad_map[a.TM - 1][tnb - 1][wave] : 0u;
+  const int m0 = (int)(wm & 7u), an = (int)(wm >> 3 & 7u), c0 = (int)(wm >> 6 & 15u);
+  auto wm_has = [&](int i) { return (wm >> (10 + i) & 1u) != 0; };
+  auto wm_c1 = [&](int i) { return (int)(wm >> (14 + 4 * i) & 15u); };
   const int K = a.K1 + a.K2;
 
   f32x16 acc[4][2];
@@ -509,19 +517,23 @@
     H = __builtin_bit_cast(bf16x8, p[0]); M = __builtin_bit_cast(bf16x8, p[64]); L = __builtin_bit_cast(bf16x8, p[128]);
   };
   auto consume = [&](int cur) {
-    if (an > 0 && kn > 0) {
+    if (an > 0) {
       bf16x8 Bh0, Bm0, Bl0, Bh1, Bm1, Bl1;
-      rdfrag(cur, ASLOTS + 2 * wp, Bh0, Bm0, Bl0);
-      if (kn > 1) rdfrag(cur, ASLOTS + 2 * wp + 1, Bh1, Bm1, Bl1);
-      else { Bh1 = Bh0; Bm1 = Bm0; Bl1 = Bl0; }
+      rdfrag(cur, ASLOTS + c0, Bh0, Bm0, Bl0);
+      Bh1 = Bh0; Bm1 = Bm0; Bl1 = Bl0;
+      int c1 = -1;
       bf16x8 An[3];
       rdfrag(cur, m0, An[0], An[1], An[2]);
 #pragma unroll
       for (int i = 0; i < 4; ++i) {
         if (i < an) {
           const bf16x8 Ah = An[0], Am = An[1], Al = An[2];
+          if (wm_has(i) && wm_c1(i) != c1) {
+            c1 = wm_c1(i);
+            rdfrag(cur, ASLOTS + c1, Bh1, Bm1, Bl1);
+          }
           if (i + 1 < an) rdfrag(cur, m0 + i + 1, An[0], An[1], An[2]);
-          if (kn > 1) {
+          if (wm_has(i)) {
             x3_chain2(acc[i][0], acc[i][1], Ah, Am, Al, Bh0, Bm0, Bl0, Ah, Am, Al, Bh1, Bm1, Bl1);
           } else {
             x3_chain(acc[i][0], Ah, Am, Al, Bh0, Bm0, Bl0);
@@ -563,11 +575,12 @@
   for (int i = 0; i < 4; ++i)
 #pragma unroll
     for (int j = 0; j < 2; ++j)
-      if (i < an && j < kn) {
+      if (i < an && (j == 0 || wm_has(i))) {
+        const int ct = tn0 + (j == 0 ? c0 : wm_c1(i));
 #pragma unroll
         for (int r = 0; r < 16; ++r) {
           const int row = (m0 + i) * 32 + (r & 3) + 8 * (r >> 2) + 4 * lh;
-          out[(int64_t)row * ldw + (tn0 + 2 * wp + j) * 32 + li] = acc[i][j][r];
+          out[(int64_t)row * ldw + ct * 32 + li] = acc[i][j][r];
         }
       }
 }
diff --git a/mr-gnas_amd/csrc/wgrad_map.hpp b/mr-gnas_amd/csrc/wgrad_map.hpp
--- /dev/null
+++ b/mr-gnas_amd/csrc/wgrad_map.hpp
@@ -0,0 +1,132 @@
+#pragma once
+#ifndef WGRAD_MAP_STORAGE
+#define WGRAD_MAP_STORAGE static const
+#endif
+WGRAD_MAP_STORAGE unsigned wgrad_map[7][16][8] = {
+  {
+    {0x00000008u, 0x00000000u, 0x00000000u, 0x00000000u, 0x00000000u, 0x00000000u, 0x00000000u, 0x00000000u},
+    {0x00000008u, 0x00000048u, 0x00000000u, 0x00000000u, 0x00000000u, 0x00000000u, 0x00000000u, 0x00000000u},
+    {0x00000008u, 0x00000048u, 0x00000088u, 0x00000000u, 0x00000000u, 0x00000000u, 0x00000000u, 0x00000000u},
+    {0x00000008u, 0x00000048u, 0x00000088u, 0x000000c8u, 0x00000000u, 0x00000000u, 0x00000000u, 0x00000000u},
+    {0x00000008u, 0x00000048u, 0x00000088u, 0x000104c8u, 0x00000000u, 0x00000000u, 0x00000000u, 0x00000000u},
+    {0x00000008u, 0x00000048u, 0x00010488u, 0x000144c8u, 0x00000000u, 0x00000000u, 0x00000000u, 0x00000000u},
+    {0x00000008u, 0x00010448u, 0x00014488u, 0x000184c8u, 0x00000000u, 0x00000000u, 0x00000000u, 0x00000000u},
+    {0x00000008u, 0x00000048u, 0x00000088u, 0x000000c8u, 0x00000108u, 0x00000148u, 0x00000188u, 0x000001c8u},
+    {0x00000008u, 0x00000048u, 0x00000088u, 0x000000c8u, 0x00000108u, 0x00000148u, 0x00000188u, 0x000205c8u},
+    {0x00000008u, 0x00000048u, 0x00000088u, 0x000000c8u, 0x00000108u, 0x00000148u, 0x00020588u, 0x000245c8u},
+    {0x00000008u, 0x00000048u, 0x00000088u, 0x000000c8u, 0x00000108u, 0x00020548u, 0x00024588u, 0x000285c8u},
+    {0x00000008u, 0x00000048u, 0x00000088u, 0x000000c8u, 0x00020508u, 0x00024548u, 0x00028588u, 0x0002c5c8u},
+    {0x00000008u, 0x00000048u, 0x00000088u, 0x000204c8u, 0x00024508u, 0x00028548u, 0x0002c588u, 0x000305c8u},
+    {0x00000008u, 0x00000048u, 0x00020488u, 0x000244c8u, 0x00028508u, 0x0002c548u, 0x00030588u, 0x000345c8u},
+    {0x00000008u, 0x00020448u, 0x00024488u, 0x000284c8u, 0x0002c508u, 0x00030548u, 0x00034588u, 0x000385c8u},
+    {0x00020408u, 0x00024448u, 0x00028488u, 0x0002c4c8u, 0x00030508u, 0x00034548u, 0x00038588u, 0x0003c5c8u},
+  },
+  {
+    {0x00000008u, 0x00000009u, 0x00000000u, 0x00000000u, 0x00000000u, 0x00000000u, 0x00000000u, 0x00000000u},
+    {0x00000008u, 0x00000009u, 0x00000048u, 0x00000049u, 0x00000000u, 0x00000000u, 0x00000000u, 0x00000000u},
+    {0x00000010u, 0x00000050u, 0x00000088u, 0x00000089u, 0x00000000u, 0x00000000u, 0x00000000u, 0x00000000u},
+    {0x00000010u, 0x00000050u, 0x00000090u, 0x000000d0u, 0x00000000u, 0x00000000u, 0x00000000u, 0x00000000u},
+    {0x00000010u, 0x00000050u, 0x00100890u, 0x000104d0u, 0x00000000u, 0x00000000u, 0x00000000u, 0x00000000u},
+    {0x00100810u, 0x00140850u, 0x00010490u, 0x000144d0u, 0x00000000u, 0x00000000u, 0x00000000u, 0x00000000u},
+    {0x00100810u, 0x00010450u, 0x00154c90u, 0x00198cd0u, 0x00000000u, 0x00000000u, 0x00000000u, 0x00000000u},
+    {0x00000010u, 0x00000050u, 0x00000090u, 0x000000d0u, 0x00000110u, 0x00000150u, 0x00000190u, 0x000001d0u},
+    {0x00000010u, 0x00000050u, 0x00000090u, 0x000000d0u, 0x00000110u, 0x00000150u, 0x00200990u, 0x000205d0u},
+    {0x00000010u, 0x00000050u, 0x00000090u, 0x000000d0u, 0x00200910u, 0x00240950u, 0x00020590u, 0x000245d0u},
+    {0x00000010u, 0x00000050u, 0x00200890u, 0x002408d0u, 0x00280910u, 0x00020550u, 0x00024590u, 0x000285d0u},
+    {0x00200810u, 0x00240850u, 0x00280890u, 0x002c08d0u, 0x00020510u, 0x00024550u, 0x00028590u, 0x0002c5d0u},
+    {0x00200810u, 0x00240850u, 0x00280890u, 0x000204d0u, 0x00024510u, 0x00028550u, 0x002ecd90u, 0x00330dd0u},
+    {0x00200810u, 0x00240850u, 0x00020490u, 0x000244d0u, 0x002a8d10u, 0x002ecd50u, 0x00330d90u, 0x00374dd0u},
+    {0x00200810u, 0x00020450u, 0x00264c90u, 0x002a8cd0u, 0x002ecd10u, 0x00330d50u, 0x00374d90u, 0x003b8dd0u},
+    {0x00220c10u, 0x00264c50u, 0x002a8c90u, 0x002eccd0u, 0x00330d10u, 0x00374d50u, 0x003b8d90u, 0x003fcdd0u},
+  },
+  {
+    {0x00000008u, 0x00000009u, 0x0000000au, 0x00000000u, 0x00000000u, 0x00000000u, 0x00000000u, 0x00000000u},
+    {0x00000010u, 0x0000000au, 0x00000050u, 0x0000004au, 0x00000000u, 0x00000000u, 0x00000000u, 0x00000000u},
+    {0x00000018u, 0x00000050u, 0x0000004au, 0x00000090u, 0x00000000u, 0x00000000u, 0x0000008au, 0x00000000u},
+    {0x00000018u, 0x00000058u, 0x00000098u, 0x000000d8u, 0x00000000u, 0x00000000u, 0x00000000u, 0x00000000u},
+    {0x00000018u, 0x01001058u, 0x00100898u, 0x000104d8u, 0x00000000u, 0x00000000u, 0x00000000u, 0x00000000u},
+    {0x00100818u, 0x00140858u, 0x01011498u, 0x014154d8u, 0x00000000u, 0x00000000u, 0x00000000u, 0x00000000u},
+    {0x01101818u, 0x01411458u, 0x00154c98u, 0x01999cd8u, 0x00000000u, 0x00000000u, 0x00000000u, 0x00000000u},
+    {0x00000018u, 0x00000058u, 0x00000098u, 0x000000d8u, 0x00000118u, 0x00000158u, 0x00000198u, 0x000001d8u},
+    {0x00000018u, 0x00000058u, 0x00000098u, 0x000000d8u, 0x00000118u, 0x02001158u, 0x00200998u, 0x000205d8u},
+    {0x00000018u, 0x00000058u, 0x02001098u, 0x024010d8u, 0x00200918u, 0x00240958u, 0x00020598u, 0x000245d8u},
+    {0x02001018u, 0x02401058u, 0x00200898u, 0x002408d8u, 0x00280918u, 0x00020558u, 0x00024598u, 0x028295d8u},
+    {0x00200818u, 0x00240858u, 0x00280898u, 0x002c08d8u, 0x02021518u, 0x02425558u, 0x02829598u, 0x02c2d5d8u},
+    {0x00200818u, 0x02241858u, 0x02681898u, 0x028214d8u, 0x02c25518u, 0x03029558u, 0x002ecd98u, 0x00330dd8u},
+    {0x02201818u, 0x02641858u, 0x02821498u, 0x02c254d8u, 0x002a8d18u, 0x002ecd58u, 0x03331d98u, 0x03775dd8u},
+    {0x02201818u, 0x02421458u, 0x00264c98u, 0x02aa9cd8u, 0x02eedd18u, 0x03331d58u, 0x03775d98u, 0x03bb9dd8u},
+    {0x02221c18u, 0x02665c58u, 0x02aa9c98u, 0x02eedcd8u, 0x03331d18u, 0x03775d58u, 0x03bb9d98u, 0x03ffddd8u},
+  },
+  {
+    {0x00000008u, 0x00000009u, 0x0000000au, 0x0000000bu, 0x00000000u, 0x00000000u, 0x00000000u, 0x00000000u},
+    {0x00000010u, 0x00000012u, 0x00000050u, 0x00000052u, 0x00000000u, 0x00000000u, 0x00000000u, 0x00000000u},
+    {0x00000018u, 0x0000000bu, 0x00000058u, 0x0000004bu, 0x00000000u, 0x00000090u, 0x00000000u, 0x00000092u},
+    {0x00000020u, 0x00000060u, 0x000000a0u, 0x000000e0u, 0x00000000u, 0x00000000u, 0x00000000u, 0x00000000u},
+    {0x10002020u, 0x01001060u, 0x001008a0u, 0x000104e0u, 0x00000000u, 0x00000000u, 0x00000000u, 0x00000000u},
+    {0x10102820u, 0x14142860u, 0x010114a0u, 0x014154e0u, 0x00000000u, 0x00000000u, 0x00000000u, 0x00000000u},
+    {0x11103820u, 0x15413460u, 0x18156ca0u, 0x01999ce0u, 0x00000000u, 0x00000000u, 0x00000000u, 0x00000000u},
+    {0x00000020u, 0x00000060u, 0x000000a0u, 0x000000e0u, 0x00000120u, 0x00000160u, 0x000001a0u, 0x000001e0u},
+    {0x00000020u, 0x00000060u, 0x000000a0u, 0x000000e0u, 0x20002120u, 0x02001160u, 0x002009a0u, 0x000205e0u},
+    {0x20002020u, 0x24002060u, 0x020010a0u, 0x024010e0u, 0x00200920u, 0x00240960u, 0x000205a0u, 0x000245e0u},
+    {0x02001020u, 0x02401060u, 0x002008a0u, 0x002408e0u, 0x20282920u, 0x24022560u, 0x280265a0u, 0x028295e0u},
+    {0x20202820u, 0x24242860u, 0x282828a0u, 0x2c2c28e0u, 0x02021520u, 0x02425560u, 0x028295a0u, 0x02c2d5e0u},
+    {0x20202820u, 0x02241860u, 0x026818a0u, 0x028214e0u, 0x26c27520u, 0x2b02b560u, 0x2c2eeda0u, 0x30332de0u},
+    {0x22203820u, 0x26643860u, 0x2a8234a0u, 0x2ec274e0u, 0x302aad20u, 0x342eed60u, 0x03331da0u, 0x03775de0u},
+    {0x22203820u, 0x26423460u, 0x28266ca0u, 0x02aa9ce0u, 0x2eeefd20u, 0x33333d60u, 0x37777da0u, 0x3bbbbde0u},
+    {0x22223c20u, 0x26667c60u, 0x2aaabca0u, 0x2eeefce0u, 0x33333d20u, 0x37777d60u, 0x3bbbbda0u, 0x3ffffde0u},
+  },
+  {
+    {0x00000010u, 0x0000000au, 0x0000000bu, 0x0000000cu, 0x00000000u, 0x00000000u, 0x00000000u, 0x00000000u},
+    {0x00000018u, 0x00000013u, 0x00000058u, 0x00000053u, 0x00000000u, 0x00000000u, 0x00000000u, 0x00000000u},
+    {0x00000020u, 0x0000000cu, 0x00000060u, 0x0000004cu, 0x00000000u, 0x00000098u, 0x00000000u, 0x00000093u},
+    {0x00000020u, 0x00000060u, 0x000000a0u, 0x000000e0u, 0x0000000cu, 0x0000004cu, 0x0000008cu, 0x000000ccu},
+    {0x10002020u, 0x01001060u, 0x001008a0u, 0x000104e0u, 0x0000000cu, 0x0000004cu, 0x0000008cu, 0x000104ccu},
+    {0x10102820u, 0x14142860u, 0x010114a0u, 0x014154e0u, 0x0000000cu, 0x0000004cu, 0x0001048cu, 0x000144ccu},
+    {0x11103820u, 0x15413460u, 0x18156ca0u, 0x01999ce0u, 0x0000000cu, 0x0001044cu, 0x0001448cu, 0x000184ccu},
+    {0x11113c20u, 0x15557c60u, 0x1999bca0u, 0x1dddfce0u, 0x0001040cu, 0x0001444cu, 0x0001848cu, 0x0001c4ccu},
+    {0x00000000u, 0x00000000u, 0x00000000u, 0x00000000u, 0x00000000u, 0x00000000u, 0x00000000u, 0x00000000u},
+    {0x00000000u, 0x00000000u, 0x00000000u, 0x00000000u, 0x00000000u, 0x00000000u, 0x00000000u, 0x00000000u},
+    {0x00000000u, 0x00000000u, 0x00000000u, 0x00000000u, 0x00000000u, 0x00000000u, 0x00000000u, 0x00000000u},
+    {0x00000000u, 0x00000000u, 0x00000000u, 0x00000000u, 0x00000000u, 0x00000000u, 0x00000000u, 0x00000000u},
+    {0x00000000u, 0x00000000u, 0x00000000u, 0x00000000u, 0x00000000u, 0x00000000u, 0x00000000u, 0x00000000u},
+    {0x00000000u, 0x00000000u, 0x00000000u, 0x00000000u, 0x00000000u, 0x00000000u, 0x00000000u, 0x00000000u},
+    {0x00000000u, 0x00000000u, 0x00000000u, 0x00000000u, 0x00000000u, 0x00000000u, 0x00000000u, 0x00000000u},
+    {0x00000000u, 0x00000000u, 0x00000000u, 0x00000000u, 0x00000000u, 0x00000000u, 0x00000000u, 0x00000000u},
+  },
+  {
+    {0x00000010u, 0x00000012u, 0x0000000cu, 0x0000000du, 0x00000000u, 0x00000000u, 0x00000000u, 0x00000000u},
+    {0x00000018u, 0x0000001bu, 0x00000058u, 0x0000005bu, 0x00000000u, 0x00000000u, 0x00000000u, 0x00000000u},
+    {0x00000020u, 0x00000014u, 0x00000060u, 0x00000054u, 0x00000088u, 0x00000099u, 0x00000000u, 0x00000094u},
+    {0x00000020u, 0x00000060u, 0x000000a0u, 0x000000e0u, 0x00000014u, 0x00000054u, 0x00000094u, 0x000000d4u},
+    {0x10002020u, 0x01001060u, 0x001008a0u, 0x000104e0u, 0x00000014u, 0x00000054u, 0x00100894u, 0x000104d4u},
+    {0x10102820u, 0x14142860u, 0x010114a0u, 0x014154e0u, 0x00100814u, 0x00140854u, 0x00010494u, 0x000144d4u},
+    {0x11103820u, 0x15413460u, 0x18156ca0u, 0x01999ce0u, 0x00100814u, 0x00010454u, 0x00154c94u, 0x00198cd4u},
+    {0x11113c20u, 0x15557c60u, 0x1999bca0u, 0x1dddfce0u, 0x00110c14u, 0x00154c54u, 0x00198c94u, 0x001dccd4u},
+    {0x00000000u, 0x00000000u, 0x00000000u, 0x00000000u, 0x00000000u, 0x00000000u, 0x00000000u, 0x00000000u},
+    {0x00000000u, 0x00000000u, 0x00000000u, 0x00000000u, 0x00000000u, 0x00000000u, 0x00000000u, 0x00000000u},
+    {0x00000000u, 0x00000000u, 0x00000000u, 0x00000000u, 0x00000000u, 0x00000000u, 0x00000000u, 0x00000000u},
+    {0x00000000u, 0x00000000u, 0x00000000u, 0x00000000u, 0x00000000u, 0x00000000u, 0x00000000u, 0x00000000u},
+    {0x00000000u, 0x00000000u, 0x00000000u, 0x00000000u, 0x00000000u, 0x00000000u, 0x00000000u, 0x00000000u},
+    {0x00000000u, 0x00000000u, 0x00000000u, 0x00000000u, 0x00000000u, 0x00000000u, 0x00000000u, 0x00000000u},
+    {0x00000000u, 0x00000000u, 0x00000000u, 0x00000000u, 0x00000000u, 0x00000000u, 0x00000000u, 0x00000000u},
+    {0x00000000u, 0x00000000u, 0x00000000u, 0x00000000u, 0x00000000u, 0x00000000u, 0x00000000u, 0x00000000u},
+  },
+  {
+    {0x00000010u, 0x00000012u, 0x00000014u, 0x0000000eu, 0x00000000u, 0x00000000u, 0x00000000u, 0x00000000u},
+    {0x00000020u, 0x0000001cu, 0x00000060u, 0x0000005cu, 0x00000000u, 0x00000000u, 0x00000000u, 0x00000000u},
+    {0x00000020u, 0x0000001cu, 0x00000060u, 0x0000005cu, 0x00000090u, 0x00000092u, 0x0000008cu, 0x00000095u},
+    {0x00000020u, 0x00000060u, 0x000000a0u, 0x000000e0u, 0x0000001cu, 0x0000005cu, 0x0000009cu, 0x000000dcu},
+    {0x10002020u, 0x01001060u, 0x001008a0u, 0x000104e0u, 0x0000001cu, 0x0100105cu, 0x0010089cu, 0x000104dcu},
+    {0x10102820u, 0x14142860u, 0x010114a0u, 0x014154e0u, 0x0010081cu, 0x0014085cu, 0x0101149cu, 0x014154dcu},
+    {0x11103820u, 0x15413460u, 0x18156ca0u, 0x01999ce0u, 0x0110181cu, 0x0141145cu, 0x00154c9cu, 0x01999cdcu},
+    {0x11113c20u, 0x15557c60u, 0x1999bca0u, 0x1dddfce0u, 0x01111c1cu, 0x01555c5cu, 0x01999c9cu, 0x01dddcdcu},
+    {0x00000000u, 0x00000000u, 0x00000000u, 0x00000000u, 0x00000000u, 0x00000000u, 0x00000000u, 0x00000000u},
+    {0x00000000u, 0x00000000u, 0x00000000u, 0x00000000u, 0x00000000u, 0x00000000u, 0x00000000u, 0x00000000u},
+    {0x00000000u, 0x00000000u, 0x00000000u, 0x00000000u, 0x00000000u, 0x00000000u, 0x00000000u, 0x00000000u},
+    {0x00000000u, 0x00000000u, 0x00000000u, 0x00000000u, 0x00000000u, 0x00000000u, 0x00000000u, 0x00000000u},
+    {0x00000000u, 0x00000000u, 0x00000000u, 0x00000000u, 0x00000000u, 0x00000000u, 0x00000000u, 0x00000000u},
+    {0x00000000u, 0x00000000u, 0x00000000u, 0x00000000u, 0x00000000u, 0x00000000u, 0x00000000u, 0x00000000u},
+    {0x00000000u, 0x00000000u, 0x00000000u, 0x00000000u, 0x00000000u, 0x00000000u, 0x00000000u, 0x00000000u},
+    {0x00000000u, 0x00000000u, 0x00000000u, 0x00000000u, 0x00000000u, 0x00000000u, 0x00000000u, 0x00000000u},
+  },
+};
diff --git a/mr-gnas_amd/csrc/x3_parts.hpp b/mr-gnas_amd/csrc/x3_parts.hpp
--- a/mr-gnas_amd/csrc/x3_parts.hpp
+++ b/mr-gnas_amd/csrc/x3_parts.hpp
@@ -99,9 +99,11 @@
 };
 constexpr int X3Q_HT = 7;
 constexpr int X3Q_NT = 2 * X3Q_HT;
+constexpr int X3Q_NT_MIN = X3Q_NT - 1;
+inline int x3q_tiles(int N) { const int t = (N + 15) / 16; return t < X3Q_NT_MIN ? X3Q_NT_MIN : t; }
 struct BSplitTiles16 {
-  static __host__ __device__ int chunks(int nslab) { return nslab * X3Q_NT * 64; }
-  static __host__ __device__ int tiles(int) { return X3Q_NT; }
+  static __host__ __device__ int chunks(int ntile, int nslab) { return nslab * ntile * 64; }
+  static __host__ __device__ int tiles(int ntile, int) { return ntile; }
   static __device__ __forceinline__ void source(int lane, int tile, int slab, int& n, int& k0) {
     n = tile * 16 + (lane & 15); k0 = slab * 32 + (lane >> 4) * 8;
   }
@@ -157,7 +159,7 @@
 inline void launch_bsplitq3(const float* const* B, int64_t sn, int64_t sk, int N, int K, void* const* out, int count, hipStream_t st,
                             const float* const* B2 = nullptr, int ksplit = 0) {
   const int nslab = x3q_slabs(K);
-  launch_bsplit_layout<BSplitTiles16>(B, sn, sk, N, K, out, count, st, B2, ksplit, nslab);
+  launch_bsplit_layout<BSplitTiles16>(B, sn, sk, N, K, out, count, st, B2, ksplit, x3q_tiles(N), nslab);
 }
 
 __device__ __forceinline__ void wait_vmcnt(int n) {
@@ -207,9 +209,9 @@
   asm volatile("global_load_dwordx4 %0, %1, off" : "=v"(x[0]) : "v"(p0));
   asm volatile("global_load_dwordx4 %0, %1, off" : "=v"(x[1]) : "v"(p1));
 }
-template <int NCH>
+template <int NCH, int NW = 4>
 __device__ __forceinline__ void x3_fetch_b(const char* __restrict__ src, char* __restrict__ dst, const int& wave, const int& lane) {
-  constexpr int NBW = (NCH + 3) / 4;
+  constexpr int NBW = (NCH + NW - 1) / NW;
 #pragma unroll
   for (int i = 0; i < NBW; ++i) {
     int c = wave * NBW + i;
```
